# BenTheBacker/galvanise_zero

Hardware: AMD Instinct MI355X
Metric: self-play games/sec + NN leaf-evals/sec, breakthrough 8x8 @ 800 playouts/move (higher is better)
Workload: dtype bf16x3 split (hi+lo bf16 operands, ~16-bit significand, 3 MFMAs per product, fp32 accumulate)

## Files before the change

### galvanise_zero_amd/csrc/nn/forward_kernel.h

```cpp
#pragma once

#include <hip/hip_runtime.h>
#include <stdint.h>

#include <utility>

namespace gznn {

constexpr int kMaxRoles = 4;
constexpr int kMaxSegments = 32;
constexpr int kHeadBoards = 4;
constexpr int kMaxSE = 128;

struct Segment {
    int row0;
    const float* planes;
    float* pol[kMaxRoles];
    float* val;
};

typedef __attribute__((ext_vector_type(8))) __bf16 bf16x8;
typedef __attribute__((ext_vector_type(4))) float f32x4;

struct KParams {
    const __bf16* w0;
    const __bf16* w0lo;
    const float* b0;
    const __bf16* wres;
    const float* bres;
    const float* wh;
    const float* bh;
    const float* pd[kMaxRoles];
    const float* pb[kMaxRoles];
    const float* vhw;
    const float* vhb;
    const float* vdw;
    const float* vdb;
    const float* pre;
    const float* sew1;
    const float* sew2;
    float* feat;
    f32x4* resid;
    int n;
    int nseg;
    Segment seg[kMaxSegments];
    unsigned long long* stamps;
    int C, K0, B, R, VH, V, leaky, flatten_nchw, maxP, npos;
    int lgrow;
    int heads_seq;
    int H, W, wmagic;
    int value_sigmoid;
    int logits;
    int gemm_heads;
    const __bf16* pdp[kMaxRoles];
    int pkt;
    float* glog;
    int plog;
    int v2;
    int k0taps;
    int init_act;
    int S;
    int gapF;
    int FS;
    int btab_off;
    int se_off;
    int P[kMaxRoles];
    int VK;
    int cal;
    const float* wcl;
    const float* bcl;
    int cal_off;
    int nofuse;
};

__host__ __device__ constexpr int align16(int x) { return (x + 15) & ~15; }

template <int BPW, int NT = 256, bool BLOCKED = false>
__device__ __forceinline__ void dense_heads(const KParams& kp, const float* fk, float* lg, int board0, int nb);

constexpr int kMaxPTN = 23;
struct Board {
    int H, W, npos, wmagic;
    int tapmask[kMaxPTN];
    __device__ __forceinline__ int row(int p) const { return (p * wmagic) >> 16; }
};

constexpr bool kLoopSI = false;
constexpr bool kLoDirect = true;
constexpr bool kEpiInConv = false;

#ifndef GZ_STORE_SWAP
#define GZ_STORE_SWAP 0
#endif
constexpr bool kStoreSwap = GZ_STORE_SWAP != 0;

#ifndef GZ_H2_RING_VGPRS
#define GZ_H2_RING_VGPRS 128
#endif

__host__ __device__ constexpr int ring_depth(int nst, int ks, int ct, int cap) {
    const int cand[5] = {9, 6, 4, 3, 2};
    for (int i = 0; i < 5; ++i)
        if (nst % cand[i] == 0 && cand[i] * ks * ct * 4 <= cap && (cand[i] - 1) * ks * ct <= 60) return cand[i];
    return 1;
}

__host__ __device__ constexpr int gcd_c(int a, int b) { return b == 0 ? a : gcd_c(b, a % b); }
__host__ __device__ constexpr int lcm_c(int a, int b) { return a / gcd_c(a, b) * b; }

template <int F, int PTN, int NB = 1, int P = 1, int WG = 1>
struct Geo {
    static constexpr int P2 = P == 3 ? 2 : 1;
    static constexpr int WP = P == 1 ? 1 : 2;
    static constexpr int NPOS = 16 * PTN;
    static constexpr int PT = PTN;
    static constexpr int TT = NB * PT;
    static constexpr int NWV = WG == 3 ? 8 : (WG == 4 || WG == 5) ? 2 : 4;
    static constexpr int NGR = WG == 2 || WG == 4 || WG == 5 ? 2 : 1;
    static constexpr int CT = F / (16 * NWV);
    static constexpr int KC = F / 32;
    static constexpr int CPR = F / 8;
    static constexpr bool WRAP = CPR >= 16 && (P2 == 2 || PTN > 11);
    static constexpr int HALF = WRAP ? CPR * 16 : ((CPR + 14) * 16 + 255) & ~255;
    static constexpr int ROWS = WRAP ? P2 * HALF + 32 : P2 * HALF;
    static constexpr int ZROWS = WRAP ? 2 : 1;
    static constexpr int ACT_BYTES = (NPOS + ZROWS + 1) * ROWS;
    static constexpr int KS = (CT >= 4 || WP == 2) ? 1 : 2;
    static constexpr int NFR = CT * WP;
    static constexpr int ROWB = 64 * WP;
    static constexpr int NST = 9 * KC / KS;
    static constexpr int R0 = (P2 == 2 && (NB == 2 || WG == 2 || WG == 4 || WG == 5) && (KC / KS) >= 3 && NST % (KC / KS) == 0 &&
                               (KC / KS) * KS * NFR * 4 <= (WG == 4 ? GZ_H2_RING_VGPRS : WG == 5 ? 64 : 96))
                                  ? KC / KS
                                  : ring_depth(NST, KS, NFR, CT >= 4 ? 64 : 96);
    static constexpr int LIVE_VGPRS = R0 * KS * NFR * 4 + 2 * TT * P2 * 4 + 2 * CT * TT * 4;
    static constexpr bool SI = 2 * NB * ACT_BYTES + 16 * 1024 > 160 * 1024 || (NB == 1 && LIVE_VGPRS > 330) || P == 2;
    static constexpr int RS = ring_depth(NST, KS, NFR, 64);
    static constexpr int US = lcm_c(RS, KC / KS) * ((lcm_c(RS, KC / KS) * KS) % 2 ? 2 : 1);
    static constexpr bool LOOPSI = (kLoopSI || PTN > 11) && SI && NST % US == 0 && NST / US >= 2;
    static constexpr int R = LOOPSI ? RS : R0;
    static constexpr int LPS = KS * NFR;
    static constexpr bool INPL = WG == 5;
    static constexpr bool RG = CT * TT * 4 * 2 > 256;
    static constexpr bool TRACKED = SI || LIVE_VGPRS > 300 || (P2 == 2 && (NB == 2 || WG == 2 || WG == 4 || WG == 5));
    static_assert(F % 64 == 0, "filters must be a multiple of 64");
    static_assert(!SI || NB == 1, "single-image mode takes one board per workgroup");
    static_assert(WG == 1 || ((WG == 2 || WG == 4 || WG == 5) && NB == 1 && !SI) || (WG == 3 && !SI && CT >= 1),
                  "wave groups: two images, or one in place (INPL), never the single-image conv and heads");
    static_assert(!INPL || (P == 3 && WRAP), "in place: the split F = 128 kernels");
    static_assert(!RG || SI, "the global residual is implemented for single-image kernels");
    static constexpr int RESID_BYTES = RG ? 4 * CT * TT * 64 * 16 : 0;
    static constexpr int LO_BYTES = P == 2 ? ACT_BYTES : 0;
    static_assert(KC % KS == 0, "a stage must not straddle a tap");
    static_assert(R >= 2, "no ring depth fits");
    static constexpr int SPT = KC / KS;
    static constexpr int U0 = lcm_c(R, SPT);
    static constexpr int U = (U0 * KS) % 2 ? 2 * U0 : U0;
    static constexpr int NIT = NST / U;
    static constexpr int TPI = U * KS / KC;
    static constexpr bool LOOP = !SI && NST % U == 0 && NIT >= 2;
    static_assert(!LOOPSI || (NST % U == 0 && NIT >= 2), "single-image looped conv");
};

__device__ __forceinline__ int swz(int q) { return (2 * q) & 14; }

__host__ __device__ inline int trunk_scratch_bytes(int npos, int C, int K0, int R, int P2, int F) {
    const int in_stage = align16(C * npos * 4) + P2 * align16((npos + 1) * K0 * 2);
    const int hc = 2 * R + 1;
    const int heads = align16((F / 16) * hc * npos * 4);
    return in_stage > heads ? in_stage : heads;
}
__host__ __device__ inline int bias_table_bytes(int F, int B) { return align16((2 * B) * F * 4); }
__host__ __device__ inline int se_scratch_bytes(int F, int NB, int S) { return align16(NB * (F + S) * 4); }

__device__ __forceinline__ float act_fn(float v, int leaky) {
    return v > 0.f ? v : (leaky ? 0.03f * v : 0.f);
}
__device__ __forceinline__ float act_mx(float v, float alpha) { return fmaxf(v, alpha * v); }

__device__ __forceinline__ uint32_t pack2(float a, float b) {
    __bf16 x = (__bf16)a, y = (__bf16)b;
    return (uint32_t)__builtin_bit_cast(uint16_t, x) | ((uint32_t)__builtin_bit_cast(uint16_t, y) << 16);
}

__device__ __forceinline__ float bf16_lo(float x) { return x - (float)(__bf16)x; }

template <int F, int PTN, int P = 1, bool SEL = true>
__device__ __forceinline__ void store_act(char* X, int p, int co, f32x4 v, int npos) {
    using G = Geo<F, PTN, 1, P>;
    if constexpr (SEL && G::WRAP && kStoreSwap) {
        const int q = p >= npos ? npos + G::ZROWS : p;
        const uint32_t h0 = pack2(v[0], v[1]), h1 = pack2(v[2], v[3]);
        const uint32_t l0 = pack2(bf16_lo(v[0]), bf16_lo(v[1])), l1 = pack2(bf16_lo(v[2]), bf16_lo(v[3]));
        const auto s0 = __builtin_amdgcn_permlane16_swap(h0, l0, false, false);
        const auto s1 = __builtin_amdgcn_permlane16_swap(h1, l1, false, false);
        char* a = X + q * G::ROWS + ((co >> 3) << 4) + ((co & 4) ? G::HALF : 0);
        *(uint4*)a = uint4{s0[0], s1[0], s0[1], s1[1]};
        return;
    }
    if (SEL || p < npos) {
        const int q = SEL && p >= npos ? npos + G::ZROWS : p;
        const int chunk = G::WRAP ? (co >> 3) : ((co >> 3) + swz(q));
        char* a = X + q * G::ROWS + (chunk << 4) + (co & 7) * 2;
        uint2 u;
        if constexpr (P == 2) {
            u.x = pack2(bf16_lo(v[0]), bf16_lo(v[1]));
            u.y = pack2(bf16_lo(v[2]), bf16_lo(v[3]));
        } else {
            u.x = pack2(v[0], v[1]);
            u.y = pack2(v[2], v[3]);
        }
        *(uint2*)a = u;
        if constexpr (G::P2 == 2) {
            uint2 l;
            l.x = pack2(bf16_lo(v[0]), bf16_lo(v[1]));
            l.y = pack2(bf16_lo(v[2]), bf16_lo(v[3]));
            *(uint2*)(a + G::HALF) = l;
        }
    }
}

template <int F, int PTN>
__device__ __forceinline__ void store_lo_scratch(char* xlo, int p, int co, f32x4 v, int npos) {
    using G = Geo<F, PTN, 1, 2>;
    if (p < npos) {
        const int chunk = G::WRAP ? (co >> 3) : (co >> 3) + swz(p);
        uint2 l;
        l.x = pack2(bf16_lo(v[0]), bf16_lo(v[1]));
        l.y = pack2(bf16_lo(v[2]), bf16_lo(v[3]));
        *(uint2*)(xlo + p * G::ROWS + (chunk << 4) + (co & 7) * 2) = l;
    }
}

__device__ __forceinline__ float wave_sum(float v) {
#pragma unroll
    for (int o = 32; o > 0; o >>= 1) v += __shfl_xor(v, o, 64);
    return v;
}

__device__ __forceinline__ float wave_max(float v) {
#pragma unroll
    for (int o = 32; o > 0; o >>= 1) v = fmaxf(v, __shfl_xor(v, o, 64));
    return v;
}

__device__ __forceinline__ int find_segment(const KParams& kp, int board) {
    int s = 0;
    while (s + 1 < kp.nseg && board >= kp.seg[s + 1].row0) ++s;
    return s;
}

template <int IMM>
__device__ __forceinline__ bf16x8 gload_issue(uint32_t voff, const void* sbase) {
    bf16x8 v;
    asm volatile("global_load_dwordx4 %0, %1, %2 offset:%3" : "=v"(v) : "v"(voff), "s"(sbase), "n"(IMM) : "memory");
    return v;
}
template <int N>
__device__ __forceinline__ void ring_wait() { asm volatile("s_waitcnt vmcnt(%0)" ::"n"(N) : "memory"); }
__device__ __forceinline__ void ring_ready(bf16x8& v) { asm volatile("" : "+v"(v)); }


template <int F, int PTN, int NB, int P, int WG = 1>
struct Ring {
    using G = Geo<F, PTN, NB, P, WG>;
    bf16x8 r[G::R][G::KS][G::NFR];
};

template <int WP, int ROWB, int FR>
struct FragOff {
    static_assert(ROWB == 64 * WP, "16 rows x ROWB bytes = WP fragments of 1 KB");
    static constexpr int value = FR * 1024;
};
template <int F, int PTN, int NB, int P, int WG, int SLOT, int PARTS, int FR>
__device__ __forceinline__ void ring_issue_f(Ring<F, PTN, NB, P, WG>& ring, int k, uint32_t woff, const char* sb) {
    using G = Geo<F, PTN, NB, P, WG>;
    if constexpr ((PARTS >> (FR % G::WP)) & 1) {
        if constexpr (G::TRACKED)
            ring.r[SLOT][k][FR] = *(const bf16x8*)(sb + woff + FragOff<G::WP, G::ROWB, FR>::value);
        else
            ring.r[SLOT][k][FR] = gload_issue<FragOff<G::WP, G::ROWB, FR>::value>(woff, sb);
    }
}
template <int F, int PTN, int NB, int P, int WG, int SLOT, int PARTS, int... FRS>
__device__ __forceinline__ void ring_issue_k(Ring<F, PTN, NB, P, WG>& ring, int k, uint32_t woff, const char* sb,
                                             std::integer_sequence<int, FRS...>) {
    (ring_issue_f<F, PTN, NB, P, WG, SLOT, PARTS, FRS>(ring, k, woff, sb), ...);
}
template <int F, int PTN, int NB, int P, int WG, int SLOT, int PARTS = 3>
__device__ __forceinline__ void ring_issue(Ring<F, PTN, NB, P, WG>& ring, const __bf16* wres, uint32_t woff, int gs, int gmax) {
    using G = Geo<F, PTN, NB, P, WG>;
    int s = gs < gmax ? gs : gmax;
    if constexpr (P == 2) s = (s / (2 * G::NST)) * G::NST + s % G::NST;
#pragma unroll
    for (int k = 0; k < G::KS; ++k)
        ring_issue_k<F, PTN, NB, P, WG, SLOT, PARTS>(ring, k, woff, (const char*)wres + (size_t)(s * G::KS + k) * F * G::ROWB,
                                                    std::make_integer_sequence<int, G::NFR>{});
}

__device__ __forceinline__ void launder(int& v) { asm volatile("" : "+v"(v)); }
template <typename T>
__device__ __forceinline__ void launder_ptr(T*& p) { asm volatile("" : "+v"(p)); }
struct TapAddr {
    int row, rot;
};
template <int F, int PTN, int P = 1>
__device__ __forceinline__ TapAddr tap_base(int tap, int pt, int lane, const Board& bd) {
    using G = Geo<F, PTN, 1, P>;
    const int li = lane & 15, g = lane >> 4;
    const int dy = tap / 3 - 1, dx = tap % 3 - 1;
    const int p = 16 * pt + li;
    static_assert(PTN <= kMaxPTN, "board larger than the tap masks");
    const int qv = p + (dy * bd.W + dx);
    const bool ok = (bd.tapmask[pt] >> tap) & 1;
    if constexpr (G::WRAP) {
        const int a_in = qv * G::ROWS + (g << 4);
        const int a_zero = bd.npos * G::ROWS + (((g + swz(qv)) & 15) << 4);
        const int m = -(int)ok;
        return TapAddr{(a_in & m) | (a_zero & ~m), 0};
    }
    const int rot = (g + swz(qv)) << 4;
    return TapAddr{(ok ? qv : bd.npos) * G::ROWS, rot};
}
template <int F, int PTN, int P = 1>
__device__ __forceinline__ int tap_offset(const TapAddr& t, int kc) {
    return t.row + t.rot + 64 * kc;
}

template <int F, int PTN, int NB, int P, int WG, int PASS, int ST>
__device__ __forceinline__ void conv_stage(const char* __restrict__ X, Ring<F, PTN, NB, P, WG>& ring,
                                           f32x4 (&acc)[Geo<F, PTN, NB, P, WG>::CT][Geo<F, PTN, NB, P, WG>::TT],
                                           bf16x8 (&b)[2][Geo<F, PTN, NB, P, WG>::TT][Geo<F, PTN, NB, P, WG>::P2],
                                           const __bf16* wres, uint32_t woff, int gs0, int gmax, int& lane,
                                           const Board& bd) {
    using G = Geo<F, PTN, NB, P, WG>;
    constexpr int R = G::R, KS = G::KS, CT = G::CT, PT = G::PT, TT = G::TT, KC = G::KC, P2 = G::P2, WP = G::WP;
    constexpr bool next_in_pass = ST + R - 1 < G::NST;
    constexpr bool hi_only = P == 2 && G::TRACKED && (next_in_pass ? PASS == 1 : PASS == 0);
    ring_issue<F, PTN, NB, P, WG, (ST + R - 1) % R, hi_only ? 1 : 3>(ring, wres, woff, gs0 + ST + R - 1, gmax);
    if constexpr (!G::TRACKED) {
        ring_wait<(R - 1) * G::LPS>();
#pragma unroll
        for (int k = 0; k < KS; ++k)
#pragma unroll
            for (int f = 0; f < G::NFR; ++f) ring_ready(ring.r[ST % R][k][f]);
    }

#pragma unroll
    for (int k = 0; k < KS; ++k) {
        const int j = ST * KS + k;
        if (j + 1 < 9 * KC) {
            const int jn = j + 1;
            const int tap = jn / KC, kc = jn % KC;
            if (kc == 0) launder(lane);
#pragma unroll
            for (int pt = 0; pt < PT; ++pt) {
                const char* a = X + tap_offset<F, PTN, P>(tap_base<F, PTN, P>(tap, pt, lane, bd), kc);
#pragma unroll
                for (int bb = 0; bb < NB; ++bb)
#pragma unroll
                    for (int h = 0; h < P2; ++h)
                        b[jn & 1][bb * PT + pt][h] = *(const bf16x8*)(a + bb * G::ACT_BYTES + h * G::HALF);
            }
        }
#pragma unroll
        for (int ct = 0; ct < CT; ++ct)
#pragma unroll
            for (int t = 0; t < TT; ++t) {
                const bf16x8 w_hi = ring.r[ST % R][k][ct * WP];
                acc[ct][t] = __builtin_amdgcn_mfma_f32_16x16x32_bf16(w_hi, b[j & 1][t][0], acc[ct][t], 0, 0, 0);
                if constexpr (P == 3) {
                    const bf16x8 w_lo = ring.r[ST % R][k][ct * WP + 1];
                    acc[ct][t] = __builtin_amdgcn_mfma_f32_16x16x32_bf16(w_hi, b[j & 1][t][1], acc[ct][t], 0, 0, 0);
                    acc[ct][t] = __builtin_amdgcn_mfma_f32_16x16x32_bf16(w_lo, b[j & 1][t][0], acc[ct][t], 0, 0, 0);
                } else if constexpr (P == 2 && PASS == 0) {
                    const bf16x8 w_lo = ring.r[ST % R][k][ct * WP + 1];
                    acc[ct][t] = __builtin_amdgcn_mfma_f32_16x16x32_bf16(w_lo, b[j & 1][t][0], acc[ct][t], 0, 0, 0);
                }
            }
        if constexpr (!G::SI) {
#pragma unroll
            for (int t = 0; t < TT; ++t) {
                __builtin_amdgcn_sched_group_barrier(0x008, CT * (P2 == 2 ? 3 : 1), 0);
                __builtin_amdgcn_sched_group_barrier(0x100, P2, 0);
            }
        }
        __builtin_amdgcn_sched_barrier(0);
    }
}

template <int F, int PTN, int NB, int P, int WG, int... S>
__device__ __forceinline__ void ring_prime(Ring<F, PTN, NB, P, WG>& ring, const __bf16* wres, uint32_t woff, int gmax,
                                           std::integer_sequence<int, S...>) {
    (ring_issue<F, PTN, NB, P, WG, S>(ring, wres, woff, S, gmax), ...);
}

template <int F, int PTN, int NB, int P, int WG, int PASS, int... ST>
__device__ __forceinline__ void conv_stages(const char* __restrict__ X, Ring<F, PTN, NB, P, WG>& ring,
                                            f32x4 (&acc)[Geo<F, PTN, NB, P, WG>::CT][Geo<F, PTN, NB, P, WG>::TT],
                                            bf16x8 (&b)[2][Geo<F, PTN, NB, P, WG>::TT][Geo<F, PTN, NB, P, WG>::P2],
                                            const __bf16* wres, uint32_t woff, int gs0, int gmax, int& lane,
                                            const Board& bd, std::integer_sequence<int, ST...>) {
    (conv_stage<F, PTN, NB, P, WG, PASS, ST>(X, ring, acc, b, wres, woff, gs0, gmax, lane, bd), ...);
}

template <int F, int PTN, int NB, int P, int WG = 1, int PASS = 0>
__device__ __forceinline__ void conv3x3(const char* __restrict__ X, Ring<F, PTN, NB, P, WG>& ring,
                                        f32x4 (&acc)[Geo<F, PTN, NB, P, WG>::CT][Geo<F, PTN, NB, P, WG>::TT],
                                        const __bf16* wres, uint32_t woff, int gs0, int gmax, int lane,
                                        const Board& bd) {
    using G = Geo<F, PTN, NB, P, WG>;
    constexpr int PT = G::PT, TT = G::TT;
    if constexpr (PASS == 0) {
#pragma unroll
        for (int ct = 0; ct < G::CT; ++ct)
#pragma unroll
            for (int t = 0; t < TT; ++t) acc[ct][t] = f32x4{0.f, 0.f, 0.f, 0.f};
    }
    bf16x8 b[2][TT][G::P2];
    launder(lane);
#pragma unroll
    for (int pt = 0; pt < PT; ++pt) {
        const char* a = X + tap_offset<F, PTN, P>(tap_base<F, PTN, P>(0, pt, lane, bd), 0);
#pragma unroll
        for (int bb = 0; bb < NB; ++bb)
#pragma unroll
            for (int h = 0; h < G::P2; ++h) b[0][bb * PT + pt][h] = *(const bf16x8*)(a + bb * G::ACT_BYTES + h * G::HALF);
    }
    conv_stages<F, PTN, NB, P, WG, PASS>(X, ring, acc, b, wres, woff, gs0, gmax, lane, bd,
                                     std::make_integer_sequence<int, G::NST>{});
}

__device__ __forceinline__ void mfma_split3(f32x4& acc, const bf16x8& wh, const bf16x8& bh, const bf16x8& bl,
                                            const bf16x8& wl) {
    asm volatile(
        "v_mfma_f32_16x16x32_bf16 %0, %1, %2, %0\n\t"
        "v_mfma_f32_16x16x32_bf16 %0, %1, %3, %0\n\t"
        "v_mfma_f32_16x16x32_bf16 %0, %4, %2, %0"
        : "+a"(acc)
        : "v"(wh), "v"(bh), "v"(bl), "v"(wl));
}
template <int CT, int TT>
__device__ __forceinline__ void split_chain_enter(f32x4 (&acc)[CT][TT]) {
#pragma unroll
    for (int ct = 0; ct < CT; ++ct)
#pragma unroll
        for (int t = 0; t < TT; ++t) asm volatile("" : "+a"(acc[ct][t]));
    asm volatile("s_nop 1" ::: "memory");
}
template <int CT, int TT>
__device__ __forceinline__ void split_chain_leave(f32x4 (&acc)[CT][TT]) {
    asm volatile("s_nop 15\n\ts_nop 7" ::: "memory");
#pragma unroll
    for (int ct = 0; ct < CT; ++ct)
#pragma unroll
        for (int t = 0; t < TT; ++t) asm volatile("" : "+a"(acc[ct][t]));
}

struct NoEpi {
    __device__ __forceinline__ void operator()(int) const {}
};

template <int CT, int TT>
__device__ __forceinline__ void tile_leave(f32x4 (&acc)[CT][TT], int t) {
    asm volatile("s_nop 15\n\ts_nop 3" ::: "memory");
#pragma unroll
    for (int ct = 0; ct < CT; ++ct) asm volatile("" : "+a"(acc[ct][t]));
}

template <int F, int PTN, int NB, int P, int WG, int PASS, int ST, bool EPI = false, class Epi = NoEpi>
__device__ __forceinline__ void conv_stage_l(const char* __restrict__ X, Ring<F, PTN, NB, P, WG>& ring,
                                             f32x4 (&acc)[Geo<F, PTN, NB, P, WG>::CT][Geo<F, PTN, NB, P, WG>::TT],
                                             bf16x8 (&b)[Geo<F, PTN, NB, P, WG>::TT][Geo<F, PTN, NB, P, WG>::P2],
                                             const __bf16* wres, uint32_t woff, int gs_it, int gmax, int& lane,
                                             const Board& bd, int tap0, bool last_it, const Epi& epi = Epi{}) {
    using G = Geo<F, PTN, NB, P, WG>;
    constexpr int R = G::R, KS = G::KS, CT = G::CT, PT = G::PT, KC = G::KC, P2 = G::P2, WP = G::WP;
    static_assert(P != 2 || G::TRACKED, "two-pass split: compiler-tracked weight loads");
    static_assert(G::U % R == 0, "ring slots must be static within an iteration");
    if constexpr (P == 2) {
        constexpr int SLOT = (ST + R - 1) % R;
        const int gs = gs_it + ST + R - 1;
        ring_issue<F, PTN, NB, P, WG, SLOT, 1>(ring, wres, woff, gs, gmax);
        if constexpr (ST + R - 1 < G::U) {
            if constexpr (PASS == 0) ring_issue<F, PTN, NB, P, WG, SLOT, 2>(ring, wres, woff, gs, gmax);
        } else if ((PASS == 0) != last_it) {
            ring_issue<F, PTN, NB, P, WG, SLOT, 2>(ring, wres, woff, gs, gmax);
        }
    } else {
        ring_issue<F, PTN, NB, P, WG, (ST + R - 1) % R>(ring, wres, woff, gs_it + ST + R - 1, gmax);
    }
    if constexpr (!G::TRACKED) {
        ring_wait<(R - 1) * G::LPS>();
#pragma unroll
        for (int k = 0; k < KS; ++k)
#pragma unroll
            for (int f = 0; f < G::NFR; ++f) ring_ready(ring.r[ST % R][k][f]);
    }
#pragma unroll
    for (int k = 0; k < KS; ++k) {
        const int jn = ST * KS + k + 1;
        const int tap = tap0 + jn / KC, kc = jn % KC;
        if (kc == 0) launder(lane);
        int nb_off[PT];
#pragma unroll
        for (int pt = 0; pt < PT; ++pt) nb_off[pt] = tap_offset<F, PTN, P>(tap_base<F, PTN, P>(tap, pt, lane, bd), kc);
#pragma unroll
        for (int bb = 0; bb < NB; ++bb)
#pragma unroll
            for (int pt = 0; pt < PT; ++pt) {
                const int t = bb * PT + pt;
#pragma unroll
                for (int ct = 0; ct < CT; ++ct) {
                    const bf16x8 w_hi = ring.r[ST % R][k][ct * WP];
                    if constexpr (P2 == 2) {
                        mfma_split3(acc[ct][t], w_hi, b[t][0], b[t][1], ring.r[ST % R][k][ct * WP + 1]);
                    } else {
                        acc[ct][t] = __builtin_amdgcn_mfma_f32_16x16x32_bf16(w_hi, b[t][0], acc[ct][t], 0, 0, 0);
                        if constexpr (P == 2 && PASS == 0) {
                            const bf16x8 w_lo = ring.r[ST % R][k][ct * WP + 1];
                            acc[ct][t] = __builtin_amdgcn_mfma_f32_16x16x32_bf16(w_lo, b[t][0], acc[ct][t], 0, 0, 0);
                        }
                    }
                }
                {
                    const char* a = X + nb_off[pt] + bb * G::ACT_BYTES;
#pragma unroll
                    for (int h = 0; h < P2; ++h) b[t][h] = *(const bf16x8*)(a + h * G::HALF);
                }
                if constexpr (P2 == 1) {
                    __builtin_amdgcn_sched_group_barrier(0x008, CT * (P == 2 && PASS == 0 ? 2 : 1), 0);
                    __builtin_amdgcn_sched_group_barrier(0x100, P2, 0);
                }
                if constexpr (EPI && ST == G::U - 1) {
                    if (k == KS - 1 && t >= 1) {
                        if constexpr (P2 == 2) tile_leave(acc, t - 1);
                        epi(t - 1);
                    }
                }
            }
        if constexpr (EPI && ST == G::U - 1) {
            if (k == KS - 1) {
                if constexpr (P2 == 2) tile_leave(acc, G::TT - 1);
                epi(G::TT - 1);
            }
        }
        __builtin_amdgcn_sched_barrier(0);
    }
}

template <int F, int PTN, int NB, int P, int WG, int PASS, bool EPI, class Epi, int... ST>
__device__ __forceinline__ void conv_iter(const char* __restrict__ X, Ring<F, PTN, NB, P, WG>& ring,
                                          f32x4 (&acc)[Geo<F, PTN, NB, P, WG>::CT][Geo<F, PTN, NB, P, WG>::TT],
                                          bf16x8 (&b)[Geo<F, PTN, NB, P, WG>::TT][Geo<F, PTN, NB, P, WG>::P2],
                                          const __bf16* wres, uint32_t woff, int gs_it, int gmax, int& lane,
                                          const Board& bd, int tap0, bool last_it, const Epi& epi,
                                          std::integer_sequence<int, ST...>) {
    (conv_stage_l<F, PTN, NB, P, WG, PASS, ST, EPI, Epi>(X, ring, acc, b, wres, woff, gs_it, gmax, lane, bd, tap0, last_it,
                                                         epi), ...);
}

template <int F, int PTN, int NB, int P, int WG = 1, int PASS = 0, bool EPI = false, class Epi = NoEpi>
__device__ __forceinline__ void conv3x3_looped(const char* __restrict__ X, Ring<F, PTN, NB, P, WG>& ring,
                                               f32x4 (&acc)[Geo<F, PTN, NB, P, WG>::CT][Geo<F, PTN, NB, P, WG>::TT],
                                               const __bf16* wres, uint32_t woff, int gs0, int gmax, int lane,
                                               const Board& bd, const Epi& epi = Epi{}) {
    using G = Geo<F, PTN, NB, P, WG>;
    constexpr int PT = G::PT, TT = G::TT;
    if constexpr (PASS == 0) {
#pragma unroll
        for (int ct = 0; ct < G::CT; ++ct)
#pragma unroll
            for (int t = 0; t < TT; ++t) acc[ct][t] = f32x4{0.f, 0.f, 0.f, 0.f};
    }
    bf16x8 b[TT][G::P2];
    launder(lane);
#pragma unroll
    for (int pt = 0; pt < PT; ++pt) {
        const char* a = X + tap_offset<F, PTN, P>(tap_base<F, PTN, P>(0, pt, lane, bd), 0);
#pragma unroll
        for (int bb = 0; bb < NB; ++bb)
#pragma unroll
            for (int h = 0; h < G::P2; ++h) b[bb * PT + pt][h] = *(const bf16x8*)(a + bb * G::ACT_BYTES + h * G::HALF);
    }
    if constexpr (G::P2 == 2) split_chain_enter(acc);
    constexpr int NLOOP = EPI ? G::NIT - 1 : G::NIT;
#pragma clang loop unroll(disable)
    for (int it = 0; it < NLOOP; ++it)
        conv_iter<F, PTN, NB, P, WG, PASS, false, NoEpi>(X, ring, acc, b, wres, woff, gs0 + it * G::U, gmax, lane, bd,
                                                       it * G::TPI, it == G::NIT - 1, NoEpi{},
                                                       std::make_integer_sequence<int, G::U>{});
    if constexpr (EPI)
        conv_iter<F, PTN, NB, P, WG, PASS, true, Epi>(X, ring, acc, b, wres, woff, gs0 + NLOOP * G::U, gmax, lane, bd,
                                                   NLOOP * G::TPI, true, epi, std::make_integer_sequence<int, G::U>{});
    if constexpr (G::P2 == 2) split_chain_leave(acc);
}

template <int F, int PTN, int NB, int P, int WG = 1>
__device__ __forceinline__ f32x4 board_channel_sum(const f32x4 (&acc)[Geo<F, PTN, NB, P, WG>::CT][Geo<F, PTN, NB, P, WG>::TT],
                                                   int ct, int bb, int li, int npos) {
    using G = Geo<F, PTN, NB, P, WG>;
    f32x4 s = {0.f, 0.f, 0.f, 0.f};
#pragma unroll
    for (int pt = 0; pt < G::PT; ++pt)
        if (16 * pt + li < npos) {
            const f32x4 v = acc[ct][bb * G::PT + pt];
            s[0] += v[0]; s[1] += v[1]; s[2] += v[2]; s[3] += v[3];
        }
#pragma unroll
    for (int o = 1; o < 16; o <<= 1)
#pragma unroll
        for (int r = 0; r < 4; ++r) s[r] += __shfl_xor(s[r], o, 64);
    return s;
}

template <int F, int PTN, int NB, int P, bool ADDB>
__device__ __forceinline__ void se_gates(const KParams& kp,
                                         const f32x4 (&acc)[Geo<F, PTN, NB, P>::CT][Geo<F, PTN, NB, P>::TT],
                                         const float* bt, int blk, float* ses, int co_base, int lane,
                                         f32x4 (&gate)[Geo<F, PTN, NB, P>::CT][NB]) {
    using G = Geo<F, PTN, NB, P>;
    constexpr int CT = G::CT, PT = G::PT;
    const int g = lane >> 4, li = lane & 15, npos = kp.npos, S = kp.S;
    float* mean = ses;
    float* hid = ses + NB * F;
    const float inv = 1.f / (float)npos;
#pragma unroll
    for (int bb = 0; bb < NB; ++bb)
#pragma unroll
        for (int ct = 0; ct < CT; ++ct) {
            f32x4 s;
            if constexpr (ADDB) {
                const float4 bias = *(const float4*)(bt + co_base + 16 * ct + 4 * g);
                s = f32x4{0.f, 0.f, 0.f, 0.f};
#pragma unroll
                for (int pt = 0; pt < PT; ++pt)
                    if (16 * pt + li < npos) {
                        f32x4 v = acc[ct][bb * PT + pt];
                        v[0] += bias.x; v[1] += bias.y; v[2] += bias.z; v[3] += bias.w;
                        s[0] += v[0]; s[1] += v[1]; s[2] += v[2]; s[3] += v[3];
                    }
#pragma unroll
                for (int o = 1; o < 16; o <<= 1)
#pragma unroll
                    for (int r = 0; r < 4; ++r) s[r] += __shfl_xor(s[r], o, 64);
            } else {
                s = board_channel_sum<F, PTN, NB, P>(acc, ct, bb, li, npos);
            }
            if (li == 0)
                *(float4*)(mean + bb * F + co_base + 16 * ct + 4 * g) =
                    make_float4(s[0] * inv, s[1] * inv, s[2] * inv, s[3] * inv);
        }
    __syncthreads();
    const float* w1 = kp.sew1 + (size_t)blk * F * S;
    for (int i = threadIdx.x; i < NB * S; i += 256) {
        const int bb = i / S, j = i - bb * S;
        float h = 0.f;
#pragma unroll 16
        for (int c = 0; c < F; ++c) h += mean[bb * F + c] * w1[c * S + j];
        hid[bb * S + j] = fmaxf(h, 0.f);
    }
    __syncthreads();
    const float* w2 = kp.sew2 + (size_t)blk * S * F;
    f32x4 z[CT][NB];
#pragma unroll
    for (int ct = 0; ct < CT; ++ct)
#pragma unroll
        for (int bb = 0; bb < NB; ++bb) z[ct][bb] = f32x4{0.f, 0.f, 0.f, 0.f};
    const float* w2l = w2 + co_base + 4 * g;
#pragma unroll 4
    for (int j = 0; j < S; ++j) {
        float4 w[CT];
#pragma unroll
        for (int ct = 0; ct < CT; ++ct) w[ct] = *(const float4*)(w2l + (size_t)j * F + 16 * ct);
#pragma unroll
        for (int bb = 0; bb < NB; ++bb) {
            const float h = hid[bb * S + j];
#pragma unroll
            for (int ct = 0; ct < CT; ++ct) {
                z[ct][bb][0] += h * w[ct].x; z[ct][bb][1] += h * w[ct].y;
                z[ct][bb][2] += h * w[ct].z; z[ct][bb][3] += h * w[ct].w;
            }
        }
    }
#pragma unroll
    for (int ct = 0; ct < CT; ++ct)
#pragma unroll
        for (int bb = 0; bb < NB; ++bb)
            gate[ct][bb] = f32x4{1.f / (1.f + __expf(-z[ct][bb][0])), 1.f / (1.f + __expf(-z[ct][bb][1])),
                                 1.f / (1.f + __expf(-z[ct][bb][2])), 1.f / (1.f + __expf(-z[ct][bb][3]))};
}

template <int F, int PTN, int NB, int P>
__device__ __forceinline__ void squeeze_excite(const KParams& kp,
                                               f32x4 (&acc)[Geo<F, PTN, NB, P>::CT][Geo<F, PTN, NB, P>::TT], int blk,
                                               float* ses, int co_base, int lane) {
    using G = Geo<F, PTN, NB, P>;
    constexpr int CT = G::CT, PT = G::PT;
    f32x4 gate[CT][NB];
    se_gates<F, PTN, NB, P, false>(kp, acc, nullptr, blk, ses, co_base, lane, gate);
#pragma unroll
    for (int ct = 0; ct < CT; ++ct)
#pragma unroll
        for (int bb = 0; bb < NB; ++bb)
#pragma unroll
            for (int pt = 0; pt < PT; ++pt) {
                f32x4& v = acc[ct][bb * PT + pt];
                v[0] *= gate[ct][bb][0]; v[1] *= gate[ct][bb][1]; v[2] *= gate[ct][bb][2]; v[3] *= gate[ct][bb][3];
            }
}

__device__ __forceinline__ f32x4 pre_act(f32x4 v, const float4& sc, const float4& sh, int leaky) {
    v[0] = act_fn(v[0] * sc.x + sh.x, leaky);
    v[1] = act_fn(v[1] * sc.y + sh.y, leaky);
    v[2] = act_fn(v[2] * sc.z + sh.z, leaky);
    v[3] = act_fn(v[3] * sc.w + sh.w, leaky);
    return v;
}

template <int F, int PTN, bool LD>
__device__ __forceinline__ void lo_copy(char* X, char* xlo, int npos, int tid) {
    using G = Geo<F, PTN, 1, 2>;
    const int n16 = npos * G::ROWS / 16;
    uint4* img = (uint4*)X;
    uint4* glo = (uint4*)xlo;
    if constexpr (LD) {
        const int lane = tid & 63;
        for (int i0 = tid - lane; i0 < n16; i0 += 256) {
            if (i0 + lane < n16)
                __builtin_amdgcn_global_load_lds((const __attribute__((address_space(1))) void*)(glo + i0 + lane),
                                                 (__attribute__((address_space(3))) void*)(img + i0), 16, 0, 0);
        }
        asm volatile("s_waitcnt vmcnt(0)" ::: "memory");
    } else {
#pragma unroll 4
        for (int i = tid; i < n16; i += 256) glo[i] = img[i];
    }
}
template <int F, int PTN>
__device__ __forceinline__ void save_lo_write_hi(char* X, char* xlo, const f32x4 (&acc)[Geo<F, PTN, 1, 2>::CT][Geo<F, PTN, 1, 2>::TT],
                                                 int npos, int tid, int co_base, int li, int g) {
    using G = Geo<F, PTN, 1, 2>;
    lo_copy<F, PTN, false>(X, xlo, npos, tid);
    asm volatile("s_waitcnt lgkmcnt(0)\n\ts_barrier" ::: "memory");
#pragma unroll
    for (int ct = 0; ct < G::CT; ++ct)
#pragma unroll
        for (int t = 0; t < G::TT; ++t) store_act<F, PTN, 1, false>(X, 16 * t + li, co_base + 16 * ct + 4 * g, acc[ct][t], npos);
    __syncthreads();
}

template <int F, int PTN, int NB, int WPE, int P, bool V2, int WG = 1>
__device__ __forceinline__ void trunk_body(const KParams& kp) {
    using G = Geo<F, PTN, NB, P, WG>;
    static_assert(P == 1 || (P == 3 && (NB == 1 || G::WRAP) && (G::CT * G::TT <= 16 || G::SI)) || (P == 2 && G::SI && (!V2 || kLoDirect)),
                  "split precision: F <= 128 (F = 256: single image)");
    constexpr int P2 = G::P2;
    constexpr int IP2 = G::WP;
    constexpr int PT = G::PT, TT = G::TT, CT = G::CT, R = G::R, NWV = G::NWV, NGR = G::NGR, kThreads = 64 * NWV;
    const int NPOS = kp.npos, H = kp.H, W = kp.W;
    Board bd{H, W, NPOS, kp.wmagic, {}};
    {
        const int li = threadIdx.x & 15;
#pragma unroll
        for (int pt = 0; pt < PT; ++pt) {
            const int p = 16 * pt + li;
            const int r = bd.row(p), x = p - r * W;
            int m = 0;
#pragma unroll
            for (int tap = 0; tap < 9; ++tap) {
                const int y = r + tap / 3 - 1, xx = x + tap % 3 - 1;
                if (p < NPOS && (unsigned)y < (unsigned)H && (unsigned)xx < (unsigned)W) m |= 1 << tap;
            }
            bd.tapmask[pt] = m;
        }
    }
    constexpr int ACT = G::ACT_BYTES;

    constexpr bool SI = G::SI, RG = G::RG;
    extern __shared__ __attribute__((aligned(16))) char smem[];
    const int grp = NGR == 1 ? 0 : __builtin_amdgcn_readfirstlane((int)(threadIdx.x / kThreads));
    char* X0 = smem + grp * NB * ACT;
    constexpr bool INPL = G::INPL;
    char* X1 = SI ? smem : INPL ? X0 : smem + NGR * NB * ACT + grp * NB * ACT;
    char* SCR = X1;
    char* SCR0 = SI || INPL ? smem : smem + NGR * NB * ACT;
    float* btab = (float*)(smem + kp.btab_off);

    const int board0 = (blockIdx.x * NGR + grp) * NB;
    const int tid = threadIdx.x & (kThreads - 1);
#define GZ_STAMP(i) \
    if (kp.stamps && threadIdx.x == 0) kp.stamps[(size_t)blockIdx.x * 8 + (i)] = __builtin_amdgcn_s_memtime()
    GZ_STAMP(0);
    const int lane = tid & 63;
    const int wave = __builtin_amdgcn_readfirstlane(tid >> 6);
    const int g = lane >> 4, li = lane & 15;
    const int co_base = wave * (F / NWV);
    const int C = kp.C, K0 = kp.K0;

    constexpr int kPF = 4;
    const int nf4 = (C * NPOS) >> 2;
    const float* in_b[NB];
    bool vec_b[NB];
    float4 pf[NB][kPF];
#pragma unroll
    for (int bb = 0; bb < NB; ++bb) {
        const bool live = board0 + bb < kp.n;
        const int sg = find_segment(kp, board0 + bb);
        in_b[bb] = live ? kp.seg[sg].planes + (size_t)(board0 + bb - kp.seg[sg].row0) * C * NPOS : nullptr;
        vec_b[bb] = ((C * NPOS) & 3) == 0 && nf4 <= kPF * kThreads && ((uintptr_t)in_b[bb] & 15) == 0;
#pragma unroll
        for (int k = 0; k < kPF; ++k) {
            const int i4 = tid + k * kThreads;
            pf[bb][k] = (live && vec_b[bb] && i4 < nf4) ? ((const float4*)in_b[bb])[i4] : make_float4(0.f, 0.f, 0.f, 0.f);
        }
    }

    static_assert((F / NWV) % 16 == 0, "a wave's output channels are whole 16-channel weight blocks");
    const uint32_t woff = (uint32_t)((co_base >> 4) * G::WP * 1024 + 16 * lane);
    const int gmax = (P == 2 ? 4 : 2) * kp.B * G::NST - 1;
    Ring<F, PTN, NB, P, WG> ring;
    if (kp.B > 0) ring_prime<F, PTN, NB, P, WG>(ring, kp.wres, woff, gmax, std::make_integer_sequence<int, R - 1>{});

    f32x4 acc[CT][TT];
    f32x4 resid[RG ? 1 : CT][RG ? 1 : TT];
    f32x4* rg = RG ? kp.resid + ((size_t)(blockIdx.x * 4 + wave) * CT * TT) * 64 + lane : nullptr;
    char* xlo = P == 2 ? (char*)kp.resid + (size_t)gridDim.x * G::RESID_BYTES + (size_t)blockIdx.x * G::LO_BYTES : nullptr;

    float* calp = (float*)(smem + kp.cal_off);
    static_assert(!V2 || NWV == 4, "concat_all_layers partials: four waves per group");
    auto cal_partial = [&](int j, int bb, int li, int g) {
        float4 wv[CT];
#pragma unroll
        for (int ct = 0; ct < CT; ++ct) wv[ct] = *(const float4*)(kp.wcl + (size_t)j * F + co_base + 16 * ct + 4 * g);
#pragma unroll
        for (int pt = 0; pt < PT; ++pt) {
            float sum = 0.f;
#pragma unroll
            for (int ct = 0; ct < CT; ++ct) {
                const f32x4 a = acc[ct][bb * PT + pt];
                sum += a[0] * wv[ct].x;
                sum += a[1] * wv[ct].y;
                sum += a[2] * wv[ct].z;
                sum += a[3] * wv[ct].w;
            }
            sum += __shfl_xor(sum, 16, 64);
            sum += __shfl_xor(sum, 32, 64);
            const int p = 16 * pt + li;
            if (g == 0 && p < NPOS) calp[(wave * NB + bb) * NPOS + p] = sum;
        }
    };
    auto cal_reduce = [&](int j) {
        for (int i = tid; i < NB * NPOS; i += kThreads) {
            const int bb = i / NPOS, p = i - bb * NPOS;
            const int board = board0 + bb;
            if (board >= kp.n) continue;
            float sum = kp.bcl[j];
#pragma unroll
            for (int w = 0; w < 4; ++w) sum += calp[(w * NB + bb) * NPOS + p];
            kp.feat[(size_t)board * kp.FS + 2 * kp.R * NPOS + j * NPOS + p] = act_fn(sum, kp.leaky);
        }
    };

    for (int i = threadIdx.x; i < 2 * kp.B * F; i += kThreads * NGR) btab[i] = kp.bres[i];
    for (int i = tid; i < NB * G::ZROWS * G::ROWS / 4 && !INPL; i += kThreads) {
        const int bb = i / (G::ZROWS * G::ROWS / 4), j = i % (G::ZROWS * G::ROWS / 4);
        ((uint32_t*)(X0 + bb * ACT + NPOS * G::ROWS))[j] = 0u;
    }

    float* sin = (float*)SCR;
    char* IM = SCR + align16(C * NPOS * 4);
    const int imrow = K0 * 2;
    char* IMlo = IM + align16((NPOS + 1) * imrow);
    const int nch0 = K0 >> 3;
    const int imswz = ((nch0 & -nch0) < 16 ? (nch0 & -nch0) : 16) - 1;
    const int nk0 = K0 >> 5;
    auto load_w0 = [&](int s, bf16x8 (&x)[CT], bf16x8 (&xl)[CT]) {
#pragma unroll
        for (int ct = 0; ct < CT; ++ct) {
            const size_t o = ((size_t)(s * F + co_base + 16 * ct + li)) * 32 + 8 * g;
            x[ct] = *(const bf16x8*)(kp.w0 + o);
            if constexpr (IP2 == 2) xl[ct] = *(const bf16x8*)(kp.w0lo + o);
        }
    };
    bf16x8 a0[CT], alo0[CT];
    load_w0(0, a0, alo0);
#pragma unroll
    for (int bb = 0; bb < NB; ++bb) {
        const float* in = in_b[bb];
        if (vec_b[bb]) {
#pragma unroll
            for (int k = 0; k < kPF; ++k)
                if (tid + k * kThreads < nf4) ((float4*)sin)[tid + k * kThreads] = pf[bb][k];
        } else {
            for (int i = tid; i < C * NPOS; i += kThreads) sin[i] = in != nullptr ? in[i] : 0.f;
        }
        if (SI || bb == 0)
            for (int i = tid; i < IP2 * align16((NPOS + 1) * imrow) / 16; i += kThreads) ((uint4*)IM)[i] = uint4{0u, 0u, 0u, 0u};
        __syncthreads();
        const int T0 = kp.k0taps;
        for (int i = tid; i < NPOS * T0; i += kThreads) {
            int p = i, tap = 4;
            if (T0 == 9) { p = i / 9; tap = i - p * 9; }
            const int r = bd.row(p);
            const int y = r + tap / 3 - 1, x = p - r * W + tap % 3 - 1;
            if ((unsigned)y < (unsigned)H && (unsigned)x < (unsigned)W) {
                const float* src = sin + y * W + x;
                const int k0 = T0 == 9 ? tap * C : 0;
                for (int c = 0; c < C; ++c) {
                    const int k = k0 + c;
                    const int o = p * imrow + ((((k >> 3) ^ (p & imswz))) << 4) + (k & 7) * 2;
                    const float v = src[c * NPOS];
                    *(__bf16*)(IM + o) = (__bf16)v;
                    if constexpr (IP2 == 2) *(__bf16*)(IMlo + o) = (__bf16)bf16_lo(v);
                }
            }
        }
        __syncthreads();

#pragma unroll
        for (int ct = 0; ct < CT; ++ct)
#pragma unroll
            for (int pt = 0; pt < PT; ++pt) acc[ct][bb * PT + pt] = f32x4{0.f, 0.f, 0.f, 0.f};
        bf16x8 a[CT], alo[CT];
#pragma unroll
        for (int ct = 0; ct < CT; ++ct) {
            a[ct] = a0[ct];
            alo[ct] = alo0[ct];
        }
        for (int s = 0; s < nk0; ++s) {
            bf16x8 an[CT], alon[CT];
            if (s + 1 < nk0) load_w0(s + 1, an, alon);
#pragma unroll
            for (int pt = 0; pt < PT; ++pt) {
                const int p = 16 * pt + li;
                const int q = p < NPOS ? p : NPOS;
                const int o = q * imrow + ((((s * 4 + g)) ^ (q & imswz)) << 4);
                const bf16x8 bq = *(const bf16x8*)(IM + o);
#pragma unroll
                for (int ct = 0; ct < CT; ++ct) {
                    f32x4& c = acc[ct][bb * PT + pt];
                    c = __builtin_amdgcn_mfma_f32_16x16x32_bf16(a[ct], bq, c, 0, 0, 0);
                    if constexpr (IP2 == 2) {
                        const bf16x8 bql = *(const bf16x8*)(IMlo + o);
                        c = __builtin_amdgcn_mfma_f32_16x16x32_bf16(a[ct], bql, c, 0, 0, 0);
                        c = __builtin_amdgcn_mfma_f32_16x16x32_bf16(alo[ct], bq, c, 0, 0, 0);
                    }
                }
            }
            if (s + 1 < nk0) {
#pragma unroll
                for (int ct = 0; ct < CT; ++ct) {
                    a[ct] = an[ct];
                    if constexpr (IP2 == 2) alo[ct] = alon[ct];
                }
            }
        }
        if constexpr (SI || INPL) __syncthreads();
        const bool preact = V2 && kp.B > 0;
        f32x4* rg0 = rg;
        if constexpr (RG) launder_ptr(rg0);
        if constexpr (V2 && SI) {
            const bool bare = !kp.init_act;
#pragma unroll
            for (int ct = 0; ct < CT; ++ct) {
                const int co = co_base + 16 * ct + 4 * g;
                const float4 bias = *(const float4*)(kp.b0 + co);
                float4 psc = make_float4(1.f, 1.f, 1.f, 1.f), psh = make_float4(0.f, 0.f, 0.f, 0.f);
                if (preact) {
                    psc = *(const float4*)(kp.pre + co);
                    psh = *(const float4*)(kp.pre + F + co);
                }
#pragma unroll
                for (int pt = 0; pt < PT; ++pt) {
                    f32x4 v = acc[ct][bb * PT + pt];
                    v[0] += bias.x; v[1] += bias.y; v[2] += bias.z; v[3] += bias.w;
#pragma unroll
                    for (int r = 0; r < 4; ++r) {
                        const float a = act_fn(v[r], kp.leaky);
                        v[r] = ((int)bare | (int)(v[r] > 0.f)) ? v[r] : a;
                    }
                    if constexpr (RG) rg0[(ct * TT + bb * PT + pt) * 64] = v;
                    else resid[ct][bb * PT + pt] = v;
                    acc[ct][bb * PT + pt] = v;
                    const f32x4 sv = pre_act(v, psc, psh, kp.leaky);
                    if constexpr (P == 2) {
                        static_assert(P != 2 || kLoDirect, "two-pass v2: lo parts straight to the scratch");
                        store_act<F, PTN, 1, false>(X0 + bb * ACT, 16 * pt + li, co, sv, NPOS);
                        store_lo_scratch<F, PTN>(xlo, 16 * pt + li, co, sv, NPOS);
                    } else {
                        store_act<F, PTN, P, false>(X0 + bb * ACT, 16 * pt + li, co, sv, NPOS);
                    }
                }
            }
        } else
#pragma unroll
        for (int ct = 0; ct < CT; ++ct) {
            const int co = co_base + 16 * ct + 4 * g;
            const float4 bias = *(const float4*)(kp.b0 + co);
            float4 psc = make_float4(1.f, 1.f, 1.f, 1.f), psh = make_float4(0.f, 0.f, 0.f, 0.f);
            if (preact) {
                psc = *(const float4*)(kp.pre + co);
                psh = *(const float4*)(kp.pre + F + co);
            }
#pragma unroll
            for (int pt = 0; pt < PT; ++pt) {
                f32x4 v = acc[ct][bb * PT + pt];
                v[0] += bias.x; v[1] += bias.y; v[2] += bias.z; v[3] += bias.w;
                if (!V2 || kp.init_act) {
                    v[0] = act_fn(v[0], kp.leaky);
                    v[1] = act_fn(v[1], kp.leaky);
                    v[2] = act_fn(v[2], kp.leaky);
                    v[3] = act_fn(v[3], kp.leaky);
                }
                if constexpr (RG) rg0[(ct * TT + bb * PT + pt) * 64] = v;
                else resid[ct][bb * PT + pt] = v;
                acc[ct][bb * PT + pt] = v;
                if constexpr (P == 2 && kLoDirect) {
                    const f32x4 sv = preact ? pre_act(v, psc, psh, kp.leaky) : v;
                    store_act<F, PTN, 1, false>(X0 + bb * ACT, 16 * pt + li, co, sv, NPOS);
                    store_lo_scratch<F, PTN>(xlo, 16 * pt + li, co, sv, NPOS);
                } else {
                    store_act<F, PTN, P, !G::SI>(X0 + bb * ACT, 16 * pt + li, co, preact ? pre_act(v, psc, psh, kp.leaky) : v, NPOS);
                }
            }
        }
        if constexpr (V2)
            if (kp.cal) cal_partial(0, bb, li, g);
        __syncthreads();
        if constexpr (P == 2 && !kLoDirect) save_lo_write_hi<F, PTN>(X0, xlo, acc, NPOS, tid, co_base, li, g);
    }
    for (int i = tid; i < NB * G::ZROWS * G::ROWS / 4; i += kThreads) {
        const int bb = i / (G::ZROWS * G::ROWS / 4), j = i % (G::ZROWS * G::ROWS / 4);
        ((uint32_t*)(X1 + bb * ACT + NPOS * G::ROWS))[j] = 0u;
    }
    __syncthreads();
    if constexpr (V2)
        if (kp.cal) cal_reduce(0);

    GZ_STAMP(1);
    if constexpr (SI) {
        for (int cv = 0; cv < 2 * kp.B; ++cv) {
            const bool second = cv & 1;
            const float* bt = btab + cv * F;
            if constexpr (P == 2) {
                if constexpr (G::LOOPSI) conv3x3_looped<F, PTN, NB, P, WG, 0>(X0, ring, acc, kp.wres, woff, (2 * cv) * G::NST, gmax, lane, bd);
                else conv3x3<F, PTN, NB, P, WG, 0>(X0, ring, acc, kp.wres, woff, (2 * cv) * G::NST, gmax, lane, bd);
                __syncthreads();
                lo_copy<F, PTN, true>(X0, xlo, NPOS, tid);
                __syncthreads();
                if constexpr (G::LOOPSI) conv3x3_looped<F, PTN, NB, P, WG, 1>(X0, ring, acc, kp.wres, woff, (2 * cv + 1) * G::NST, gmax, lane, bd);
                else conv3x3<F, PTN, NB, P, WG, 1>(X0, ring, acc, kp.wres, woff, (2 * cv + 1) * G::NST, gmax, lane, bd);
            } else if constexpr (G::LOOPSI) {
                conv3x3_looped<F, PTN, NB, P, WG>(X0, ring, acc, kp.wres, woff, cv * G::NST, gmax, lane, bd);
            } else {
                conv3x3<F, PTN, NB, P, WG>(X0, ring, acc, kp.wres, woff, cv * G::NST, gmax, lane, bd);
            }
            __syncthreads();
            f32x4* rgc = rg;
            if constexpr (RG) launder_ptr(rgc);
            char* Xe = X0;
            launder_ptr(Xe);
            char* xloe = xlo;
            if constexpr (P == 2) launder_ptr(xloe);
            int lie = li, ge = g;
            launder(lie);
            launder(ge);
            if (V2 && second) {
                const int blk = cv >> 1;
                f32x4 gate[CT][NB];
#pragma unroll
                for (int ct = 0; ct < CT; ++ct)
#pragma unroll
                    for (int bb = 0; bb < NB; ++bb) gate[ct][bb] = f32x4{1.f, 1.f, 1.f, 1.f};
                if (kp.S)
                    se_gates<F, PTN, NB, P, true>(kp, acc, bt, blk, (float*)(smem + kp.se_off), co_base, 16 * ge + lie, gate);
                const bool more = blk + 1 < kp.B;
#pragma unroll
                for (int ct = 0; ct < CT; ++ct) {
                    const int co = co_base + 16 * ct + 4 * ge;
                    const float4 bias = *(const float4*)(bt + co);
                    float4 psc = make_float4(1.f, 1.f, 1.f, 1.f), psh = make_float4(0.f, 0.f, 0.f, 0.f);
                    if (more) {
                        psc = *(const float4*)(kp.pre + (size_t)(2 * blk + 2) * F + co);
                        psh = *(const float4*)(kp.pre + (size_t)(2 * blk + 3) * F + co);
                    }
#pragma unroll
                    for (int t = 0; t < TT; ++t) {
                        const f32x4 gt = gate[ct][t / PT];
                        f32x4 v = acc[ct][t], r;
                        v[0] += bias.x; v[1] += bias.y; v[2] += bias.z; v[3] += bias.w;
                        v[0] *= gt[0]; v[1] *= gt[1]; v[2] *= gt[2]; v[3] *= gt[3];
                        if constexpr (RG) r = rgc[(ct * TT + t) * 64];
                        else r = resid[ct][t];
                        v[0] += r[0]; v[1] += r[1]; v[2] += r[2]; v[3] += r[3];
                        if constexpr (RG) rgc[(ct * TT + t) * 64] = v;
                        else resid[ct][t] = v;
                        acc[ct][t] = v;
                        const f32x4 pv = pre_act(v, psc, psh, kp.leaky);
                        if constexpr (P == 2) {
                            store_act<F, PTN, 1, false>(Xe, 16 * t + lie, co, pv, NPOS);
                            store_lo_scratch<F, PTN>(xloe, 16 * t + lie, co, pv, NPOS);
                        } else {
                            store_act<F, PTN, P, !G::SI>(Xe, 16 * t + lie, co, pv, NPOS);
                        }
                    }
                }
                if (kp.cal)
#pragma unroll
                    for (int bb = 0; bb < NB; ++bb) cal_partial(blk + 1, bb, lie, ge);
                __syncthreads();
                if (kp.cal) cal_reduce(blk + 1);
                continue;
            }
#pragma unroll
            for (int ct = 0; ct < CT; ++ct) {
                const int co = co_base + 16 * ct + 4 * ge;
                const float4 bias = *(const float4*)(bt + co);
#pragma unroll
                for (int t = 0; t < TT; ++t) {
                    f32x4 v = acc[ct][t];
                    v[0] += bias.x; v[1] += bias.y; v[2] += bias.z; v[3] += bias.w;
                    if (second) {
                        f32x4 r;
                        if constexpr (RG) r = rgc[(ct * TT + t) * 64];
                        else r = resid[ct][t];
                        v[0] += r[0]; v[1] += r[1]; v[2] += r[2]; v[3] += r[3];
                    }
                    v[0] = act_fn(v[0], kp.leaky);
                    v[1] = act_fn(v[1], kp.leaky);
                    v[2] = act_fn(v[2], kp.leaky);
                    v[3] = act_fn(v[3], kp.leaky);
                    if (second) {
                        if constexpr (RG) rgc[(ct * TT + t) * 64] = v;
                        else resid[ct][t] = v;
                    }
                    if constexpr (P == 2 && kLoDirect) {
                        if (second) acc[ct][t] = v;
                        store_act<F, PTN, 1, false>(Xe, 16 * t + lie, co, v, NPOS);
                        store_lo_scratch<F, PTN>(xloe, 16 * t + lie, co, v, NPOS);
                    } else {
                        if (second || P == 2) acc[ct][t] = v;
                        store_act<F, PTN, P, !G::SI>(Xe, 16 * t + lie, co, v, NPOS);
                    }
                }
            }
            __syncthreads();
            if constexpr (P == 2 && !kLoDirect) save_lo_write_hi<F, PTN>(Xe, xlo, acc, NPOS, tid, co_base, lie, ge);
        }
    } else
    for (int blk = 0; blk < kp.B; ++blk) {
        const float alpha = kp.leaky ? 0.03f : 0.f;
        const float* b_a = btab + (2 * blk) * F;
        const float* b_b = b_a + F;

        static_assert(!(INPL && kEpiInConv), "an epilogue inside the conv writes the other image");
        if constexpr (!V2 && G::LOOP && kEpiInConv) {
            float4 bia[CT];
#pragma unroll
            for (int ct = 0; ct < CT; ++ct) bia[ct] = *(const float4*)(b_a + co_base + 16 * ct + 4 * g);
            auto epi1 = [&](int t) {
#pragma unroll
                for (int ct = 0; ct < CT; ++ct) {
                    f32x4 v = acc[ct][t];
                    v[0] = act_mx(v[0] + bia[ct].x, alpha);
                    v[1] = act_mx(v[1] + bia[ct].y, alpha);
                    v[2] = act_mx(v[2] + bia[ct].z, alpha);
                    v[3] = act_mx(v[3] + bia[ct].w, alpha);
                    store_act<F, PTN, P, !G::SI>(X1 + (t / PT) * ACT, 16 * (t % PT) + li, co_base + 16 * ct + 4 * g, v, NPOS);
                }
            };
            conv3x3_looped<F, PTN, NB, P, WG, 0, true>(X0, ring, acc, kp.wres, woff, (2 * blk) * G::NST, gmax, lane, bd, epi1);
            __syncthreads();
            float4 bib[CT];
#pragma unroll
            for (int ct = 0; ct < CT; ++ct) bib[ct] = *(const float4*)(b_b + co_base + 16 * ct + 4 * g);
            auto epi2 = [&](int t) {
#pragma unroll
                for (int ct = 0; ct < CT; ++ct) {
                    f32x4 v = acc[ct][t];
                    const f32x4 r = resid[ct][t];
                    v[0] = act_mx(v[0] + bib[ct].x + r[0], alpha);
                    v[1] = act_mx(v[1] + bib[ct].y + r[1], alpha);
                    v[2] = act_mx(v[2] + bib[ct].z + r[2], alpha);
                    v[3] = act_mx(v[3] + bib[ct].w + r[3], alpha);
                    resid[ct][t] = v;
                    acc[ct][t] = v;
                    store_act<F, PTN, P, !G::SI>(X0 + (t / PT) * ACT, 16 * (t % PT) + li, co_base + 16 * ct + 4 * g, v, NPOS);
                }
            };
            conv3x3_looped<F, PTN, NB, P, WG, 0, true>(X1, ring, acc, kp.wres, woff, (2 * blk + 1) * G::NST, gmax, lane, bd, epi2);
            __syncthreads();
            continue;
        }
        if constexpr (G::LOOP) conv3x3_looped<F, PTN, NB, P, WG>(X0, ring, acc, kp.wres, woff, (2 * blk) * G::NST, gmax, lane, bd);
        else conv3x3<F, PTN, NB, P, WG>(X0, ring, acc, kp.wres, woff, (2 * blk) * G::NST, gmax, lane, bd);
        if constexpr (INPL) __syncthreads();
#pragma unroll
        for (int ct = 0; ct < CT; ++ct) {
            const int co = co_base + 16 * ct + 4 * g;
            const float4 bias = *(const float4*)(b_a + co);
#pragma unroll
            for (int t = 0; t < TT; ++t) {
                f32x4 v = acc[ct][t];
                v[0] = act_mx(v[0] + bias.x, alpha);
                v[1] = act_mx(v[1] + bias.y, alpha);
                v[2] = act_mx(v[2] + bias.z, alpha);
                v[3] = act_mx(v[3] + bias.w, alpha);
                store_act<F, PTN, P, !G::SI>(X1 + (t / PT) * ACT, 16 * (t % PT) + li, co, v, NPOS);
            }
        }
        __syncthreads();

        if constexpr (G::LOOP) conv3x3_looped<F, PTN, NB, P, WG>(X1, ring, acc, kp.wres, woff, (2 * blk + 1) * G::NST, gmax, lane, bd);
        else conv3x3<F, PTN, NB, P, WG>(X1, ring, acc, kp.wres, woff, (2 * blk + 1) * G::NST, gmax, lane, bd);
        if constexpr (INPL) __syncthreads();
        if constexpr (V2) {
#pragma unroll
            for (int ct = 0; ct < CT; ++ct) {
                const float4 bias = *(const float4*)(b_b + co_base + 16 * ct + 4 * g);
#pragma unroll
                for (int t = 0; t < TT; ++t) {
                    acc[ct][t][0] += bias.x; acc[ct][t][1] += bias.y; acc[ct][t][2] += bias.z; acc[ct][t][3] += bias.w;
                }
            }
            if (kp.S) squeeze_excite<F, PTN, NB, P>(kp, acc, blk, (float*)(smem + kp.se_off), co_base, lane);
            const bool more = blk + 1 < kp.B;
#pragma unroll
            for (int ct = 0; ct < CT; ++ct) {
                const int co = co_base + 16 * ct + 4 * g;
                float4 psc = make_float4(1.f, 1.f, 1.f, 1.f), psh = make_float4(0.f, 0.f, 0.f, 0.f);
                if (more) {
                    psc = *(const float4*)(kp.pre + (size_t)(2 * blk + 2) * F + co);
                    psh = *(const float4*)(kp.pre + (size_t)(2 * blk + 3) * F + co);
                }
#pragma unroll
                for (int t = 0; t < TT; ++t) {
                    f32x4 v = acc[ct][t];
                    const f32x4 r = resid[ct][t];
                    v[0] += r[0]; v[1] += r[1]; v[2] += r[2]; v[3] += r[3];
                    resid[ct][t] = v;
                    acc[ct][t] = v;
                    if (more) store_act<F, PTN, P, !G::SI>(X0 + (t / PT) * ACT, 16 * (t % PT) + li, co, pre_act(v, psc, psh, kp.leaky), NPOS);
                }
            }
            if (kp.cal)
#pragma unroll
                for (int bb = 0; bb < NB; ++bb) cal_partial(blk + 1, bb, li, g);
            __syncthreads();
            if (kp.cal) cal_reduce(blk + 1);
            continue;
        }
#pragma unroll
        for (int ct = 0; ct < CT; ++ct) {
            const int co = co_base + 16 * ct + 4 * g;
            const float4 bias = *(const float4*)(b_b + co);
#pragma unroll
            for (int t = 0; t < TT; ++t) {
                f32x4 v = acc[ct][t];
                const f32x4 r = resid[ct][t];
                v[0] = act_mx(v[0] + bias.x + r[0], alpha);
                v[1] = act_mx(v[1] + bias.y + r[1], alpha);
                v[2] = act_mx(v[2] + bias.z + r[2], alpha);
                v[3] = act_mx(v[3] + bias.w + r[3], alpha);
                resid[ct][t] = v;
                acc[ct][t] = v;
                store_act<F, PTN, P, !G::SI>(X0 + (t / PT) * ACT, 16 * (t % PT) + li, co, v, NPOS);
            }
        }
        __syncthreads();
    }
    if constexpr (V2 && SI) {
#pragma unroll
        for (int ct = 0; ct < CT; ++ct)
#pragma unroll
            for (int t = 0; t < TT; ++t) {
                if constexpr (RG) acc[ct][t] = rg[(ct * TT + t) * 64];
                else acc[ct][t] = resid[ct][t];
            }
    }
    if (!G::TRACKED && kp.B > 0) {
        ring_wait<0>();
#pragma unroll
        for (int s = 0; s < R; ++s)
#pragma unroll
            for (int k = 0; k < G::KS; ++k)
#pragma unroll
                for (int f = 0; f < G::NFR; ++f) ring_ready(ring.r[s][k][f]);
    }

    GZ_STAMP(2);
    int lih = li, gh = g;
    if constexpr (V2 && SI) {
        launder(lih);
        launder(gh);
    }
    const int HC = 2 * kp.R + (kp.cal ? 0 : 1);
    constexpr int NT16 = F / 16;
    float* hpart = (float*)SCR;
    constexpr int kHoistHC = 5;
    constexpr bool HOIST_WH = !SI && CT <= 2;
    float4 whv[HOIST_WH ? kHoistHC : 1][CT];
    if constexpr (HOIST_WH) {
        if (HC <= kHoistHC) {
#pragma unroll
            for (int h = 0; h < kHoistHC; ++h)
#pragma unroll
                for (int ct = 0; ct < CT; ++ct)
                    if (h < HC) whv[h][ct] = *(const float4*)(kp.wh + (size_t)h * F + co_base + 16 * ct + 4 * gh);
        }
    }
    constexpr bool FUSE = !SI;
    const bool fuse = FUSE && !kp.nofuse;
    constexpr int NBW = NB * NGR;
    float* fk = (float*)(SCR0 + align16(NB * NT16 * HC * NPOS * 4));
    float* lg = fk + align16(kp.FS * NBW * 4) / 4;
    auto feat_at = [&](int bb, int k) -> float& {
        if (fuse) return fk[k * NBW + grp * NB + bb];
        return kp.feat[(size_t)(board0 + bb) * kp.FS + k];
    };
#pragma unroll
    for (int bb = 0; bb < NB; ++bb) {
        const int board = board0 + bb;
        if (kp.gapF && board < kp.n) {
            const float inv = 1.f / (float)NPOS;
#pragma unroll
            for (int ct = 0; ct < CT; ++ct) {
                const f32x4 sm = board_channel_sum<F, PTN, NB, P, WG>(acc, ct, bb, lih, NPOS);
                const int co = co_base + 16 * ct + 4 * gh;
                if (lih == 0)
#pragma unroll
                    for (int r = 0; r < 4; ++r)
                        if (co + r < kp.gapF) feat_at(bb, 2 * kp.R * NPOS + co + r) = sm[r] * inv;
            }
        }
        auto head_conv = [&](int h, const float4 (&wv)[CT]) {
#pragma unroll
            for (int pt = 0; pt < PT; ++pt) {
                const int p = 16 * pt + lih;
#pragma unroll
                for (int ct = 0; ct < CT; ++ct) {
                    const f32x4 a = acc[ct][bb * PT + pt];
                    float s = a[0] * wv[ct].x;
                    s += a[1] * wv[ct].y;
                    s += a[2] * wv[ct].z;
                    s += a[3] * wv[ct].w;
                    s += __shfl_xor(s, 16, 64);
                    s += __shfl_xor(s, 32, 64);
                    if (gh == 0 && p < NPOS) hpart[((bb * NT16 + co_base / 16 + ct) * HC + h) * NPOS + p] = s;
                }
            }
        };
        if constexpr (HOIST_WH) {
            if (HC <= kHoistHC) {
#pragma unroll
                for (int h = 0; h < kHoistHC; ++h)
                    if (h < HC) head_conv(h, whv[h]);
            }
        }
        if (!HOIST_WH || HC > kHoistHC) {
            for (int h = 0; h < HC; ++h) {
                float4 wv[CT];
#pragma unroll
                for (int ct = 0; ct < CT; ++ct) wv[ct] = *(const float4*)(kp.wh + (size_t)h * F + co_base + 16 * ct + 4 * gh);
                head_conv(h, wv);
            }
        }
    }
    __syncthreads();
    for (int i = tid; i < NB * HC * NPOS; i += kThreads) {
        const int bb = i / (HC * NPOS), hp = i - bb * (HC * NPOS);
        const int h = hp / NPOS, p = hp - h * NPOS;
        if (board0 + bb >= kp.n) continue;
        float s = kp.bh[h];
#pragma unroll
        for (int w = 0; w < NT16; ++w) s += hpart[((bb * NT16 + w) * HC + h) * NPOS + p];
        s = act_fn(s, kp.leaky);
        if (h < 2 * kp.R) {
            const int r = h >> 1, c = h & 1;
            const int idx = kp.flatten_nchw ? c * NPOS + p : p * 2 + c;
            feat_at(bb, r * 2 * NPOS + idx) = s;
        } else {
            feat_at(bb, 2 * kp.R * NPOS + kp.gapF + p) = s;
        }
    }
    __syncthreads();
    GZ_STAMP(3);
    if (fuse) {
        const int wb0 = blockIdx.x * NBW;
        const int nb = kp.n - wb0 < NBW ? kp.n - wb0 : NBW;
        dense_heads<NBW, kThreads * NGR>(kp, fk, lg, wb0, nb);
    }
    GZ_STAMP(4);
#undef GZ_STAMP
}

template <int F, int PTN, int NB, int WPE, int P>
__global__ void __launch_bounds__(256) __attribute__((amdgpu_waves_per_eu(WPE)))
trunk_kernel(const KParams kp) {
    trunk_body<F, PTN, NB, WPE, P, false>(kp);
}

template <int F, int PTN, int P>
__global__ void __launch_bounds__(512) __attribute__((amdgpu_waves_per_eu(2)))
trunk_kernel8(const KParams kp) {
    trunk_body<F, PTN, 1, 2, P, false, 2>(kp);
}

template <int F, int PTN, int P>
__global__ void __launch_bounds__(512) __attribute__((amdgpu_waves_per_eu(2)))
trunk_kernel_w8(const KParams kp) {
    trunk_body<F, PTN, 2, 2, P, false, 3>(kp);
}

template <int F, int PTN, int P>
__global__ void __launch_bounds__(256) __attribute__((amdgpu_waves_per_eu(1)))
trunk_kernel_h2(const KParams kp) {
    trunk_body<F, PTN, 1, 1, P, false, 4>(kp);
}

template <int F, int PTN, int P>
__global__ void __launch_bounds__(256) __attribute__((amdgpu_waves_per_eu(2)))
trunk_kernel_h2i(const KParams kp) {
    trunk_body<F, PTN, 1, 2, P, false, 5>(kp);
}

template <int F, int PTN, int NB, int WPE, int P>
__global__ void __launch_bounds__(256) __attribute__((amdgpu_waves_per_eu(WPE)))
trunk_kernel_v2(const KParams kp) {
    trunk_body<F, PTN, NB, WPE, P, true>(kp);
}

constexpr int kGemmSoftmaxMax = 3072;
constexpr int kDenseBlock = 64;

template <int BPW, int NT, bool BLOCKED = false>
__device__ __forceinline__ void dense_heads_seq(const KParams& kp, const float* fk, float* lg, int board0, int nb) {
    static_assert(BPW >= 1 && BPW <= 4, "one softmax wave per board");
    const int NPOS = kp.npos;
    const int LMAX = kp.lgrow;
    const int tid = threadIdx.x, lane = tid & 63, wave = tid >> 6;

    for (int r = 0; r < kp.R; ++r) {
        const int P = kp.P[r], K = 2 * NPOS;
        const float* Wd = kp.pd[r];
        const float* fr = fk + (size_t)r * 2 * NPOS * BPW;
        int lof = 0;
        for (int q = 0; q < r; ++q) lof += kp.P[q];
        if (kp.gemm_heads && P <= kGemmSoftmaxMax) {
            if (wave < nb) {
                constexpr int NV = kGemmSoftmaxMax / 64;
                const int b = wave, board = board0 + b;
                const float* l = kp.glog + (size_t)board * kp.plog + lof;
                float v[NV];
#pragma unroll
                for (int i = 0; i < NV; ++i) v[i] = lane + 64 * i < P ? l[lane + 64 * i] : -3.0e38f;
                float m = -3.0e38f;
#pragma unroll
                for (int i = 0; i < NV; ++i) m = fmaxf(m, v[i]);
                m = wave_max(m);
                float sum = 0.f;
#pragma unroll
                for (int i = 0; i < NV; ++i)
                    if (lane + 64 * i < P) sum += __expf(v[i] - m);
                sum = wave_sum(sum);
                const float inv = 1.f / sum;
                const int sg = find_segment(kp, board);
                float* out = kp.seg[sg].pol[r] + (size_t)(board - kp.seg[sg].row0) * P;
#pragma unroll
                for (int i = 0; i < NV; ++i)
                    if (lane + 64 * i < P) out[lane + 64 * i] = kp.logits ? v[i] : __expf(v[i] - m) * inv;
            }
            continue;
        }
        if (kp.gemm_heads) {
            for (int i = tid; i < nb * P; i += NT) {
                const int b = i / P, j = i - b * P;
                lg[b * LMAX + j] = kp.glog[(size_t)(board0 + b) * kp.plog + lof + j];
            }
        }
        for (int j = tid; j < P && !kp.gemm_heads; j += NT) {
            float a[BPW];
            float tot[BPW];
#pragma unroll
            for (int b = 0; b < BPW; ++b) a[b] = tot[b] = 0.f;
#pragma unroll 32
            for (int k = 0; k < K; ++k) {
                const float w = Wd[(size_t)k * ((P + 3) & ~3) + j];
#pragma unroll
                for (int b = 0; b < BPW; ++b) a[b] += fr[k * BPW + b] * w;
                if constexpr (BLOCKED)
                    if ((k & (kDenseBlock - 1)) == kDenseBlock - 1) {
#pragma unroll
                        for (int b = 0; b < BPW; ++b) { tot[b] += a[b]; a[b] = 0.f; }
                    }
            }
            if constexpr (BLOCKED) {
#pragma unroll
                for (int b = 0; b < BPW; ++b) a[b] = tot[b] + a[b];
            }
            const float bj = kp.pb[r][j];
#pragma unroll
            for (int b = 0; b < BPW; ++b) lg[b * LMAX + j] = a[b] + bj;
        }
        __syncthreads();
        if (wave < nb) {
            const int b = wave;
            const float* l = lg + b * LMAX;
            float m = -3.0e38f;
            for (int j = lane; j < P; j += 64) m = fmaxf(m, l[j]);
            m = wave_max(m);
            float sum = 0.f;
            for (int j = lane; j < P; j += 64) sum += __expf(l[j] - m);
            sum = wave_sum(sum);
            const float inv = 1.f / sum;
            const int board = board0 + b;
            const int sg = find_segment(kp, board);
            float* out = kp.seg[sg].pol[r] + (size_t)(board - kp.seg[sg].row0) * P;
            if (kp.logits) {
                for (int j = lane; j < P; j += 64) out[j] = l[j];
            } else {
                for (int j = lane; j < P; j += 64) out[j] = __expf(l[j] - m) * inv;
            }
        }
        __syncthreads();
    }

    {
        const int VH = kp.VH, VK = kp.VK;
        const float* fv = fk + (size_t)2 * kp.R * NPOS * BPW;
        for (int j = tid; j < VH; j += NT) {
            float a[BPW];
            float tot[BPW];
#pragma unroll
            for (int b = 0; b < BPW; ++b) a[b] = tot[b] = 0.f;
#pragma unroll 32
            for (int k = 0; k < VK; ++k) {
                const float w = kp.vhw[(size_t)k * ((VH + 3) & ~3) + j];
#pragma unroll
                for (int b = 0; b < BPW; ++b) a[b] += fv[k * BPW + b] * w;
                if constexpr (BLOCKED)
                    if ((k & (kDenseBlock - 1)) == kDenseBlock - 1) {
#pragma unroll
                        for (int b = 0; b < BPW; ++b) { tot[b] += a[b]; a[b] = 0.f; }
                    }
            }
            if constexpr (BLOCKED) {
#pragma unroll
                for (int b = 0; b < BPW; ++b) a[b] = tot[b] + a[b];
            }
            const float bj = kp.vhb[j];
#pragma unroll
            for (int b = 0; b < BPW; ++b) lg[b * LMAX + j] = act_fn(a[b] + bj, kp.leaky);
        }
        __syncthreads();
        if (wave < nb) {
            const int b = wave;
            const float* hv = lg + b * LMAX;
            float o[4] = {0.f, 0.f, 0.f, 0.f};
            for (int v = 0; v < kp.V; ++v) {
                float sum = 0.f;
                for (int k = lane; k < VH; k += 64) sum += hv[k] * kp.vdw[(size_t)k * kp.V + v];
                o[v] = wave_sum(sum) + kp.vdb[v];
            }
            if (lane == 0) {
                const int board = board0 + b;
                const int sg = find_segment(kp, board);
                float* out = kp.seg[sg].val + (size_t)(board - kp.seg[sg].row0) * kp.V;
                if (kp.logits) {
                    for (int v = 0; v < kp.V; ++v) out[v] = o[v];
                } else if (kp.value_sigmoid) {
                    for (int v = 0; v < kp.V; ++v) out[v] = 1.f / (1.f + __expf(-o[v]));
                } else {
                    float m = o[0];
                    for (int v = 1; v < kp.V; ++v) m = fmaxf(m, o[v]);
                    float e[4], esum = 0.f;
                    for (int v = 0; v < kp.V; ++v) { e[v] = __expf(o[v] - m); esum += e[v]; }
                    for (int v = 0; v < kp.V; ++v) out[v] = e[v] / esum;
                }
            }
        }
    }
}


template <int BPW, int NT, bool BLOCKED>
__device__ __forceinline__ void dense_heads(const KParams& kp, const float* fk, float* lg, int board0, int nb) {
    static_assert(BPW >= 1 && BPW <= 4, "one softmax wave per board");
    if (kp.heads_seq || (kp.gemm_heads && kp.maxP > kGemmSoftmaxMax)) {
        dense_heads_seq<BPW, NT, BLOCKED>(kp, fk, lg, board0, nb);
        return;
    }
    const int NPOS = kp.npos, R = kp.R, LG = kp.lgrow;
    const int tid = threadIdx.x, lane = tid & 63, wave = tid >> 6;
    const bool gem = kp.gemm_heads != 0;
    int pgroups = 0;
    if (!gem)
        for (int r = 0; r < R; ++r) pgroups += (kp.P[r] + 3) >> 2;
    const int VH4 = (kp.VH + 3) & ~3;
    const int voff = 4 * pgroups;
    const int units = pgroups + (VH4 >> 2);
    for (int u = tid; u < units; u += NT) {
        const float* W;
        const float* f;
        int K, N4, q, off, r = 0;
        if (u < pgroups) {
            int uu = u;
            off = 0;
            for (; r < R - 1; ++r) {
                const int g = (kp.P[r] + 3) >> 2;
                if (uu < g) break;
                uu -= g;
                off += 4 * g;
            }
            q = uu;
            W = kp.pd[r];
            N4 = (kp.P[r] + 3) & ~3;
            K = 2 * NPOS;
            f = fk + (size_t)r * 2 * NPOS * BPW;
        } else {
            q = u - pgroups;
            W = kp.vhw;
            N4 = VH4;
            K = kp.VK;
            f = fk + (size_t)2 * R * NPOS * BPW;
            off = voff;
        }
        float a[BPW][4];
        float tot[BPW][4];
#pragma unroll
        for (int b = 0; b < BPW; ++b) {
            a[b][0] = a[b][1] = a[b][2] = a[b][3] = 0.f;
            tot[b][0] = tot[b][1] = tot[b][2] = tot[b][3] = 0.f;
        }
        const float4* w4 = (const float4*)W + q;
        const int rs = N4 >> 2;
#pragma unroll 16
        for (int k = 0; k < K; ++k) {
            const float4 w = w4[(size_t)k * rs];
#pragma unroll
            for (int b = 0; b < BPW; ++b) {
                const float x = f[k * BPW + b];
                a[b][0] += x * w.x;
                a[b][1] += x * w.y;
                a[b][2] += x * w.z;
                a[b][3] += x * w.w;
            }
            if constexpr (BLOCKED)
                if ((k & (kDenseBlock - 1)) == kDenseBlock - 1) {
#pragma unroll
                    for (int b = 0; b < BPW; ++b)
#pragma unroll
                        for (int i = 0; i < 4; ++i) { tot[b][i] += a[b][i]; a[b][i] = 0.f; }
                }
        }
        if constexpr (BLOCKED) {
#pragma unroll
            for (int b = 0; b < BPW; ++b)
#pragma unroll
                for (int i = 0; i < 4; ++i) a[b][i] = tot[b][i] + a[b][i];
        }
        if (u < pgroups) {
#pragma unroll
            for (int i = 0; i < 4; ++i) {
                const int j = 4 * q + i;
                if (j < kp.P[r]) {
                    const float bj = kp.pb[r][j];
#pragma unroll
                    for (int b = 0; b < BPW; ++b) lg[b * LG + off + j] = a[b][i] + bj;
                }
            }
        } else {
#pragma unroll
            for (int i = 0; i < 4; ++i) {
                const int j = 4 * q + i;
                if (j < kp.VH) {
                    const float bj = kp.vhb[j];
#pragma unroll
                    for (int b = 0; b < BPW; ++b) lg[b * LG + off + j] = act_fn(a[b][i] + bj, kp.leaky);
                }
            }
        }
    }
    __syncthreads();
    const int ntask = R * nb + nb;
    for (int t = wave; t < ntask; t += NT / 64) {
        if (t < R * nb) {
            const int r = t / nb, b = t - r * nb, P = kp.P[r];
            int lof = 0;
            for (int q = 0; q < r; ++q) lof += gem ? kp.P[q] : ((kp.P[q] + 3) & ~3);
            const int board = board0 + b;
            const int sg = find_segment(kp, board);
            float* out = kp.seg[sg].pol[r] + (size_t)(board - kp.seg[sg].row0) * P;
            if (gem) {
                constexpr int NV = kGemmSoftmaxMax / 64;
                const float* l = kp.glog + (size_t)board * kp.plog + lof;
                float v[NV];
#pragma unroll
                for (int i = 0; i < NV; ++i) v[i] = lane + 64 * i < P ? l[lane + 64 * i] : -3.0e38f;
                float m = -3.0e38f;
#pragma unroll
                for (int i = 0; i < NV; ++i) m = fmaxf(m, v[i]);
                m = wave_max(m);
                float sum = 0.f;
#pragma unroll
                for (int i = 0; i < NV; ++i)
                    if (lane + 64 * i < P) sum += __expf(v[i] - m);
                sum = wave_sum(sum);
                const float inv = 1.f / sum;
#pragma unroll
                for (int i = 0; i < NV; ++i)
                    if (lane + 64 * i < P) out[lane + 64 * i] = kp.logits ? v[i] : __expf(v[i] - m) * inv;
            } else {
                const float* l = lg + b * LG + lof;
                float m = -3.0e38f;
                for (int j = lane; j < P; j += 64) m = fmaxf(m, l[j]);
                m = wave_max(m);
                float sum = 0.f;
                for (int j = lane; j < P; j += 64) sum += __expf(l[j] - m);
                sum = wave_sum(sum);
                const float inv = 1.f / sum;
                if (kp.logits) {
                    for (int j = lane; j < P; j += 64) out[j] = l[j];
                } else {
                    for (int j = lane; j < P; j += 64) out[j] = __expf(l[j] - m) * inv;
                }
            }
        } else {
            const int b = t - R * nb;
            const float* hv = lg + b * LG + voff;
            float o[4] = {0.f, 0.f, 0.f, 0.f};
            for (int v = 0; v < kp.V; ++v) {
                float sum = 0.f;
                for (int k = lane; k < kp.VH; k += 64) sum += hv[k] * kp.vdw[(size_t)k * kp.V + v];
                o[v] = wave_sum(sum) + kp.vdb[v];
            }
            if (lane == 0) {
                const int board = board0 + b;
                const int sg = find_segment(kp, board);
                float* out = kp.seg[sg].val + (size_t)(board - kp.seg[sg].row0) * kp.V;
                if (kp.logits) {
                    for (int v = 0; v < kp.V; ++v) out[v] = o[v];
                } else if (kp.value_sigmoid) {
                    for (int v = 0; v < kp.V; ++v) out[v] = 1.f / (1.f + __expf(-o[v]));
                } else {
                    float m = o[0];
                    for (int v = 1; v < kp.V; ++v) m = fmaxf(m, o[v]);
                    float e[4], esum = 0.f;
                    for (int v = 0; v < kp.V; ++v) { e[v] = __expf(o[v] - m); esum += e[v]; }
                    for (int v = 0; v < kp.V; ++v) out[v] = e[v] / esum;
                }
            }
        }
    }
}

__host__ __device__ inline int heads_row(int R, const int* P, int VH, bool two = true) {
    int maxP = 0, sum4 = 0;
    for (int r = 0; r < R; ++r) {
        maxP = P[r] > maxP ? P[r] : maxP;
        sum4 += (P[r] + 3) & ~3;
    }
    const int row = maxP > VH ? maxP : VH;
    const int tw = sum4 + ((VH + 3) & ~3);
    return two && tw > row ? tw : row;
}

__host__ __device__ inline int fused_heads_bytes(int npos, int R, int lgrow, int gapF, int nb, int nbg, int F) {
    const int FS = (2 * R + 1) * npos + gapF;
    return align16(nbg * (F / 16) * (2 * R + 1) * npos * 4) + align16(FS * nb * 4) + align16(nb * lgrow * 4);
}

#ifdef GZNN_DEFINE_HEADS_KERNEL
__global__ void __launch_bounds__(256) policy_gemm_kernel(const KParams kp) {
    const int r = blockIdx.z, P = kp.P[r], K = 2 * kp.npos;
    const int lane = threadIdx.x & 63, wave = threadIdx.x >> 6;
    const int jt0 = blockIdx.y * 8;
    const int njt = (P + 15) / 16;
    if (jt0 >= njt) return;
    const int board = blockIdx.x * 64 + wave * 16 + (lane & 15);
    const int kq = 8 * (lane >> 4);
    const float* f = kp.feat + (size_t)(board < kp.n ? board : 0) * kp.FS + (size_t)r * K;
    f32x4 acc[8];
#pragma unroll
    for (int t = 0; t < 8; ++t) acc[t] = f32x4{0.f, 0.f, 0.f, 0.f};
    const bf16x8* wp = (const bf16x8*)kp.pdp[r];
    for (int kt = 0; kt < kp.pkt; ++kt) {
        float x[8];
#pragma unroll
        for (int e = 0; e < 8; ++e) {
            const int k = 32 * kt + kq + e;
            x[e] = (board < kp.n && k < K) ? f[k] : 0.f;
        }
        bf16x8 bh, bl;
#pragma unroll
        for (int e = 0; e < 8; ++e) {
            bh[e] = (__bf16)x[e];
            bl[e] = (__bf16)(x[e] - (float)bh[e]);
        }
#pragma unroll
        for (int t = 0; t < 8; ++t) {
            const int jt = jt0 + t;
            if (jt < njt) {
                const size_t o = ((size_t)jt * kp.pkt + kt) * 128 + lane;
                const bf16x8 ah = wp[o], al = wp[o + 64];
                acc[t] = __builtin_amdgcn_mfma_f32_16x16x32_bf16(ah, bh, acc[t], 0, 0, 0);
                acc[t] = __builtin_amdgcn_mfma_f32_16x16x32_bf16(ah, bl, acc[t], 0, 0, 0);
                acc[t] = __builtin_amdgcn_mfma_f32_16x16x32_bf16(al, bh, acc[t], 0, 0, 0);
            }
        }
    }
    if (board >= kp.n) return;
    int lof = 0;
    for (int q = 0; q < r; ++q) lof += kp.P[q];
    float* out = kp.glog + (size_t)board * kp.plog + lof;
#pragma unroll
    for (int t = 0; t < 8; ++t) {
        const int j0 = (jt0 + t) * 16 + 4 * (lane >> 4);
#pragma unroll
        for (int i = 0; i < 4; ++i)
            if (j0 + i < P) out[j0 + i] = acc[t][i] + kp.pb[r][j0 + i];
    }
}

template <bool BLOCKED>
__device__ __forceinline__ void heads_body(const KParams& kp) {
    constexpr int BPW = kHeadBoards;
    extern __shared__ __attribute__((aligned(16))) float hs[];
    const int FS = kp.FS;
    float* fk = hs;
    float* lg = hs + FS * BPW;
    const int tid = threadIdx.x;
    const int board0 = blockIdx.x * BPW;
    const int nb = kp.n - board0 < BPW ? kp.n - board0 : BPW;
    for (int i0 = 0; i0 < BPW * FS; i0 += 8 * 256) {
        float r[8];
#pragma unroll
        for (int u = 0; u < 8; ++u) {
            const int i = i0 + u * 256 + tid;
            const int b = i / FS, k = i - b * FS;
            r[u] = (i < BPW * FS && b < nb) ? kp.feat[(size_t)(board0 + b) * FS + k] : 0.f;
        }
#pragma unroll
        for (int u = 0; u < 8; ++u) {
            const int i = i0 + u * 256 + tid;
            const int b = i / FS, k = i - b * FS;
            if (i < BPW * FS) fk[k * BPW + b] = r[u];
        }
    }
    __syncthreads();
    dense_heads<BPW, 256, BLOCKED>(kp, fk, lg, board0, nb);
}

__global__ void __launch_bounds__(256) heads_kernel(const KParams kp) { heads_body<false>(kp); }
__global__ void __launch_bounds__(256) heads_kernel_blocked(const KParams kp) { heads_body<true>(kp); }

#endif

__host__ inline int heads_lds_bytes(int FS, int lgrow) {
    return (FS * kHeadBoards + kHeadBoards * lgrow + kHeadBoards * 4) * 4;
}

}
```

### galvanise_zero_amd/csrc/nn/gz_nn.hip

```cpp
#define GZNN_DEFINE_HEADS_KERNEL
#include "forward_kernel.h"
#include "trunk_variants.h"
#include "fp32_forward.h"
#include "layered_forward.h"
#include "eval_cache.h"
#include "shadow_compare.h"
#include "symmetry.h"
#include "weight_image.h"
#include "../../../include/gzero_nn.h"

#include <hip/hip_runtime.h>

#include <algorithm>
#include <map>
#include <mutex>
#include <cmath>
#include <cstdio>
#include <cstdlib>
#include <cstring>
#include <string>
#include <vector>

using namespace gznn;
using namespace gzw;

static thread_local std::string g_err;

static int fail(const std::string& msg) {
    g_err = msg;
    return -1;
}

#define HIPCHK(x)                                                                        \
    do {                                                                                 \
        hipError_t e_ = (x);                                                             \
        if (e_ != hipSuccess) return fail(std::string(#x) + ": " + hipGetErrorString(e_)); \
    } while (0)


struct gz_net : PackSpec {
    int device = 0;
    size_t nweights = 0;
    struct Trunk {
        const void* fn = nullptr;
        int nb = 1;
        int smem = 0;
        int btab_off = 0;
        int se_off = 0;
        int cal_off = 0;
        bool fused_heads = false;
        int resid_bytes = 0;
        int threads = 256;
        int wgs_per_cu = 1;
        std::string name;
    } small, large;
    int large_min_rows = 1 << 30;
    bool has_weights = false;
    size_t image_bytes = 0;
    float last_roll_ms = 0.f;

    char* dmem = nullptr;
    KParams kp{};
    std::mutex wmu;
    unsigned long long wepoch = 1;

    hipStream_t stream = nullptr;
    hipEvent_t ev0 = nullptr, ev1 = nullptr;
    float* d_io = nullptr;
    int io_cap = 0;
    float last_ms = 0.f;
    int heads_smem = 0;
    std::map<hipStream_t, std::pair<float*, int>> glog;
    std::mutex feat_mu;
    std::map<hipStream_t, std::pair<float*, int>> feat;
    std::map<hipStream_t, std::pair<char*, size_t>> resid;
    unsigned long long* d_stamps = nullptr;
    int stamp_cap = 0;
    bool stamps_on = false;
    double stamp_avg[8] = {0};
    int chunk_rows = 1;
    const float* w0f = nullptr;
    const float* wresf = nullptr;
    std::map<hipStream_t, std::pair<char*, int>> fscr;
    int layered = 0;
    std::map<hipStream_t, int*> bexp;
    int in_width() const { return layered ? K0 : cp; }
    struct Shadow;
    Shadow* shadow = nullptr;
    std::mutex shadow_mu;
    bool is_shadow = false;
};

struct gz_net::Shadow {
    static constexpr int kSlots = 8;
    gz_net* net = nullptr;
    int every = 64, max_rows = 256;
    bool from_env = false;
    long forwards = 0;
    gz_shadow_stats* d_acc = nullptr;
    struct Out { float* out = nullptr; gzshadow::RowRecord* rec = nullptr; };
    std::map<hipStream_t, Out> out;
    struct Slot {
        gz_shadow_stats* host = nullptr;
        hipEvent_t e0 = nullptr, e1 = nullptr;
        bool pending = false;
        long epoch = 0;
    } slot[kSlots];
    int next = 0;
    hipStream_t last_stream = nullptr;
    int last_slot = -1;
    long epoch = 0;
    bool fresh = true;
    gz_shadow_stats done{};
};

extern "C" const char* gz_nn_last_error(void) { return g_err.c_str(); }


constexpr int kSmallVariant = 11, kLargeVariant = 23, kLargeFallback = 21, kLargeMinRows = 257;
constexpr int kLargeInPlace = 25;
constexpr int kCUs = 256;

static KernelChoice select_kernel(int fpad, int pt, int v, int precision, bool v2) {
    if (pt < 1 || pt > kMaxPT) return KernelChoice{};
    return trunk_variant(fpad, pt, v, precision, v2);
}

static gz_net* create_host(const gz_net_desc& d, int device, gz_net::Trunk* in_place) {
    if (d.cnn_kernel_size != 3) { fail("only cnn_kernel_size 3 is supported"); return nullptr; }
    if (d.role_count < 1 || d.role_count > GZ_MAX_ROLES) { fail("role_count out of range"); return nullptr; }
    if (d.num_values < 1 || d.num_values > 4) { fail("num_values out of range"); return nullptr; }
    if (initial_kernel(d) != 1 && initial_kernel(d) != 3) { fail("initial conv kernel must be 1 or 3"); return nullptr; }
    if (d.se_units < 0 || d.se_units > kMaxSE || (d.se_units && !d.resnet_v2)) {
        fail("squeeze-excite units must be 0.." + std::to_string(kMaxSE) + " on a v2 net");
        return nullptr;
    }
    if (d.concat_all_layers && (!d.resnet_v2 || d.global_pooling_value || d.value_bn)) {
        fail("concat_all_layers needs a v2 net without the pooling value head (model.py:251-252)");
        return nullptr;
    }
    const int precision = d.precision == 0 ? GZ_PRECISION_BF16 : d.precision;
    const bool fp32 = precision == GZ_PRECISION_FP32;
    const int layered = precision == GZ_PRECISION_BF16_LAYERED ? 1 : precision == GZ_PRECISION_SPLIT_LAYERED ? 3 :
                        precision == GZ_PRECISION_F16X3_LAYERED ? gzlayered::kF16Parts : 0;
    const bool layerwise = fp32 || layered;
    if (precision != GZ_PRECISION_BF16 && precision != GZ_PRECISION_SPLIT && !layerwise) { fail("unknown precision"); return nullptr; }
    int vs = kSmallVariant, vl = kLargeVariant, min_large = kLargeMinRows;
    if (const char* e = getenv("GZ_KERNEL_VARIANT")) {
        vs = vl = atoi(e);
        min_large = 1 << 30;
    }
    const int npos_ = d.input_columns * d.input_rows;
    const int pt = kernel_tiles((npos_ + 15) / 16);
    const int fpad = fp32 ? gzfp32::padded_filters(d.cnn_filter_size) : kernel_filters(d.cnn_filter_size, (npos_ + 15) / 16);
    if (d.input_rows > 32 || npos_ >= 1024) { fail("board too large"); return nullptr; }
    const bool v2 = d.resnet_v2 != 0;
    if (layerwise) {
        if (d.input_columns < 1 || d.input_rows < 1 || d.input_columns > gzfp32::kMaxBoardSide ||
            d.input_rows > gzfp32::kMaxBoardSide || fpad == 0 || d.input_channels < 1) {
            fail("unsupported network geometry F=" + std::to_string(d.cnn_filter_size) + " H=" +
                 std::to_string(d.input_columns) + " W=" + std::to_string(d.input_rows) +
                 (fp32 ? " (fp32-ieee: boards up to 19 x 19, F <= 256)" : " (layered modes: boards up to 19 x 19, F <= 256)"));
            return nullptr;
        }
        min_large = 1 << 30;
    }
    KernelChoice kc = layerwise ? KernelChoice{} : select_kernel(fpad, pt, vs, precision, v2);
    KernelChoice kl = layerwise ? KernelChoice{} : select_kernel(fpad, pt, vl, precision, v2);
    if (!kl.fn && vl == kLargeVariant) kl = select_kernel(fpad, pt, kLargeFallback, precision, v2);
    auto wg_fits = [&](const KernelChoice& c) {
        if (c.groups == 1) return true;
        const int np = d.input_columns * d.input_rows;
        const int kk0 = initial_kernel(d);
        const int k0p = ((kk0 * kk0 * d.input_channels + 31) / 32) * 32;
        const int p2 = precision == GZ_PRECISION_SPLIT ? 2 : 1;
        return trunk_scratch_bytes(np, d.input_channels, k0p, d.role_count, p2, fpad) <= c.act_bytes &&
               fused_heads_bytes(np, d.role_count, heads_row(d.role_count, d.policy_dist_count, d.value_hidden_size),
                                 gap_features(d), c.nb, 1, fpad) <= c.act_bytes;
    };
    if (kl.fn && !wg_fits(kl)) {
        kl = vl == kLargeVariant ? select_kernel(fpad, pt, kLargeFallback, precision, v2) : KernelChoice{};
        if (kl.fn && !wg_fits(kl)) kl = KernelChoice{};
    }
    if (kc.fn && !wg_fits(kc)) kc = KernelChoice{};
    KernelChoice ki = !layerwise && getenv("GZ_KERNEL_VARIANT") == nullptr && kl.fn
                          ? select_kernel(fpad, pt, kLargeInPlace, precision, v2) : KernelChoice{};
    if (ki.fn && !wg_fits(ki)) ki = KernelChoice{};
    if (kc.fn && !kl.fn && vl != vs) {
        kl = kc;
        min_large = 1 << 30;
    }
    if (!layerwise && (!kc.fn || !kl.fn)) {
        fail("unsupported network geometry F=" + std::to_string(d.cnn_filter_size) + " H=" +
             std::to_string(d.input_columns) + " W=" + std::to_string(d.input_rows) +
             (precision == GZ_PRECISION_SPLIT ? " (split precision)" : "") + (v2 ? " (v2)" : "") +
             (fpad == 256 ? " (F > 128: boards of up to 176 positions; larger boards run in fp32-ieee)" : ""));
        return nullptr;
    }
    gz_net* net = new gz_net;
    net->d = d;
    net->device = device;
    net->large_min_rows = min_large;
    static_cast<PackSpec&>(*net) = pack_spec(d, precision, fpad, false);
    net->layered = layered;
    const int k0 = initial_kernel(d);
    if (layerwise) {
        net->chunk_rows = gzfp32::chunk_rows_for(npos_, net->in_width(), fpad);
        if (const char* e = getenv("GZ_FP32_CHUNK_ROWS"))
            net->chunk_rows = std::max(1, std::min(atoi(e), net->chunk_rows));
    }
    net->nweights = blob_plan(d).consumed;
    int maxP = 0;
    for (int r = 0; r < d.role_count; ++r) maxP = std::max(maxP, d.policy_dist_count[r]);
    const int npos = d.input_columns * d.input_rows;
    int lgrow = heads_row(d.role_count, d.policy_dist_count, d.value_hidden_size, true);
    bool heads_seq = false;
    const int scr_in = trunk_scratch_bytes(npos, d.input_channels, net->K0, d.role_count, net->p2, fpad);
    auto trunk = [&](const KernelChoice& c) {
        gz_net::Trunk t;
        t.fn = c.fn;
        t.nb = c.nb;
        t.threads = c.threads;
        t.wgs_per_cu = c.wgs_per_cu;
        t.name = c.name;
        t.fused_heads = !c.single_image && !d.concat_all_layers;
        const int scr = t.fused_heads ? std::max(scr_in, fused_heads_bytes(npos, d.role_count, lgrow, gap_features(d), c.nb,
                                                                           c.groups == 2 ? 1 : c.nb, fpad))
                                      : scr_in;
        t.btab_off = c.single_image ? align16(std::max(c.act_bytes, scr))
                     : c.in_place   ? c.nb * c.act_bytes
                                    : c.nb * c.act_bytes + std::max(c.nb * c.act_bytes, scr);
        t.resid_bytes = c.resid_bytes;
        t.smem = t.btab_off + bias_table_bytes(fpad, d.residual_layers);
        t.se_off = t.smem;
        if (d.se_units) t.smem += se_scratch_bytes(fpad, c.nb, d.se_units);
        t.cal_off = t.smem;
        if (d.concat_all_layers) t.smem += align16(4 * c.nb * npos * 4);
        return t;
    };
    const int FS = 2 * d.role_count * npos + value_features(d);
    for (int pass = 0; pass < 2; ++pass) {
        net->small = trunk(kc);
        net->large = trunk(kl);
        if (layerwise) {
            gz_net::Trunk t;
            t.name = layered ? gzlayered::conv_kernel_name(fpad, layered) : gzfp32::conv_kernel_name(fpad);
            net->small = net->large = t;
        }
        net->heads_smem = heads_lds_bytes(FS, lgrow);
        if (pass == 1 || (net->small.smem <= 160 * 1024 && net->large.smem <= 160 * 1024 && net->heads_smem <= 160 * 1024))
            break;
        heads_seq = true;
        lgrow = heads_row(d.role_count, d.policy_dist_count, d.value_hidden_size, false);
    }
    net->gemm_heads = !fp32 && !net->f16 && !net->small.fused_heads && !net->large.fused_heads && maxP >= 512 &&
                      getenv("GZ_NO_GEMM_HEADS") == nullptr;
    KParams& kp = net->kp;
    kp.C = d.input_channels;
    kp.K0 = net->K0;
    kp.B = d.residual_layers;
    kp.R = d.role_count;
    kp.VH = d.value_hidden_size;
    kp.V = d.num_values;
    kp.leaky = d.leaky_relu;
    kp.flatten_nchw = d.flatten_nchw;
    kp.value_sigmoid = d.value_sigmoid;
    kp.v2 = d.resnet_v2 ? 1 : 0;
    kp.k0taps = k0 * k0;
    kp.init_act = has_initial_bn(d) ? 1 : 0;
    kp.S = d.se_units;
    kp.gapF = gap_features(d);
    kp.FS = FS;
    kp.VK = value_features(d);
    kp.cal = cal_layers(d);
    kp.nofuse = d.concat_all_layers ? 1 : 0;
    kp.maxP = maxP;
    kp.lgrow = lgrow;
    kp.heads_seq = heads_seq ? 1 : 0;
    kp.npos = npos;
    kp.gemm_heads = net->gemm_heads ? 1 : 0;
    kp.pkt = (2 * npos + 31) / 32;
    kp.plog = 0;
    for (int r = 0; r < d.role_count; ++r) kp.plog += d.policy_dist_count[r];
    kp.H = d.input_columns;
    kp.W = d.input_rows;
    kp.wmagic = (65536 + kp.W - 1) / kp.W;
    for (int r = 0; r < d.role_count; ++r) kp.P[r] = d.policy_dist_count[r];

    for (const gz_net::Trunk* t : {&net->small, &net->large}) {
        if (t->smem > 160 * 1024) {
            fail("network needs " + std::to_string(t->smem) + " B of LDS per workgroup (160 KB max): too many residual blocks "
                 "for this board in this mode");
            delete net;
            return nullptr;
        }
    }
    *in_place = ki.fn && net->large_min_rows < (1 << 30) ? trunk(ki) : gz_net::Trunk{};
    return net;
}

static gz_net* create_device(gz_net* net, const gz_net::Trunk& in_place) {
    const int device = net->device;
    if (hipSetDevice(device) != hipSuccess || hipStreamCreateWithFlags(&net->stream, hipStreamNonBlocking) != hipSuccess ||
        hipEventCreate(&net->ev0) != hipSuccess || hipEventCreate(&net->ev1) != hipSuccess) {
        fail(std::string("HIP init failed: ") + hipGetErrorString(hipGetLastError()));
        delete net;
        return nullptr;
    }
    auto resident = [&](const gz_net::Trunk& t) {
        int nblk = 0;
        if (t.smem > 64 * 1024 && hipFuncSetAttribute(t.fn, hipFuncAttributeMaxDynamicSharedMemorySize, t.smem) != hipSuccess)
            return 0;
        if (hipOccupancyMaxActiveBlocksPerMultiprocessor(&nblk, t.fn, t.threads, t.smem) != hipSuccess) return 0;
        return nblk;
    };
    if (in_place.fn) {
        const gz_net::Trunk& t = in_place;
        if (2 * t.smem <= 160 * 1024 && resident(t) >= t.wgs_per_cu) net->large = t;
    }
    for (gz_net::Trunk* t : {&net->small, &net->large}) {
        if (t->smem > 64 * 1024 &&
            hipFuncSetAttribute(t->fn, hipFuncAttributeMaxDynamicSharedMemorySize, t->smem) != hipSuccess) {
            fail("cannot raise dynamic LDS limit");
            delete net;
            return nullptr;
        }
        if (t->wgs_per_cu > 1) t->wgs_per_cu = std::max(1, std::min(t->wgs_per_cu, resident(*t)));
    }
    if (net->heads_smem > 64 * 1024 &&
        hipFuncSetAttribute(net->fp32 || net->f16 ? (const void*)&heads_kernel_blocked : (const void*)&heads_kernel,
                            hipFuncAttributeMaxDynamicSharedMemorySize, net->heads_smem) != hipSuccess) {
        fail("cannot raise dynamic LDS limit (heads)");
        delete net;
        return nullptr;
    }
    return net;
}

namespace {
int net_precision(const gz_net_desc& d) { return d.precision == 0 ? GZ_PRECISION_BF16 : d.precision; }

gz_net* shadow_host(const gz_net_desc& d, int device, int precision, int every, int max_rows, gz_net::Trunk* in_place) {
    if (precision == 0) precision = GZ_PRECISION_BF16;
    if (precision == net_precision(d)) {
        fail("shadow: precision " + std::to_string(precision) + " is the net's own mode");
        return nullptr;
    }
    if (every < 1 || max_rows < 1) {
        fail("shadow: every and max_rows must be at least 1");
        return nullptr;
    }
    gz_net_desc sd = d;
    sd.precision = precision;
    gz_net* s = create_host(sd, device, in_place);
    if (!s) {
        fail("shadow: " + g_err);
        return nullptr;
    }
    s->is_shadow = true;
    return s;
}

int shadow_env(int* precision, int* every, int* max_rows) {
    const char* e = getenv("GZ_NN_SHADOW");
    if (!e || !*e) return 0;
    long v[3] = {0, 64, 256};
    int got = 0;
    const char* p = e;
    bool ok = true;
    while (ok && got < 3) {
        char* end = nullptr;
        const long x = strtol(p, &end, 10);
        ok = end != p && x >= 0 && x <= (1 << 20);
        v[got++] = x;
        p = end;
        if (!ok || *p == 0) break;
        ok = *p == ':' && got < 3;
        ++p;
    }
    if (!ok || *p != 0 || v[1] < 1 || v[2] < 1) {
        fail(std::string("GZ_NN_SHADOW: expected <precision>[:<every>[:<max_rows>]] with every and max_rows >= 1, got \"") + e + "\"");
        return -1;
    }
    *precision = (int)v[0];
    *every = (int)v[1];
    *max_rows = (int)v[2];
    return 1;
}

void shadow_free(gz_net::Shadow* sh) {
    if (!sh) return;
    if (sh->net) gz_net_destroy(sh->net);
    if (sh->d_acc) (void)hipFree(sh->d_acc);
    for (auto& o : sh->out) (void)hipFree(o.second.out);
    for (auto& s : sh->slot) {
        if (s.host) (void)hipHostFree(s.host);
        if (s.e0) (void)hipEventDestroy(s.e0);
        if (s.e1) (void)hipEventDestroy(s.e1);
    }
    delete sh;
}

int shadow_attach(gz_net* net, gz_net* s, const gz_net::Trunk& in_place, int every, int max_rows, bool from_env) {
    if (!create_device(s, in_place)) return fail("shadow: " + g_err);
    gz_net::Shadow* sh = new gz_net::Shadow;
    sh->net = s;
    sh->every = every;
    sh->max_rows = max_rows;
    sh->from_env = from_env;
    s->kp.logits = net->kp.logits;
    hipError_t e = hipMalloc((void**)&sh->d_acc, sizeof(gz_shadow_stats));
    for (auto& sl : sh->slot) {
        if (e == hipSuccess) e = hipHostMalloc((void**)&sl.host, sizeof(gz_shadow_stats), hipHostMallocDefault);
        if (e == hipSuccess) e = hipEventCreate(&sl.e0);
        if (e == hipSuccess) e = hipEventCreate(&sl.e1);
    }
    if (e != hipSuccess) {
        shadow_free(sh);
        return fail(std::string("shadow: ") + hipGetErrorString(e));
    }
    std::lock_guard<std::mutex> wl(net->wmu);
    std::lock_guard<std::mutex> sl(net->shadow_mu);
    net->shadow = sh;
    return 0;
}

void shadow_harvest(gz_net::Shadow* sh, int wait_slot = -1) {
    if (wait_slot >= 0 && sh->slot[wait_slot].pending) (void)hipEventSynchronize(sh->slot[wait_slot].e1);
    for (int k = 0; k < gz_net::Shadow::kSlots; ++k) {
        gz_net::Shadow::Slot& s = sh->slot[(sh->next + k) % gz_net::Shadow::kSlots];
        if (!s.pending) continue;
        if (hipEventQuery(s.e1) != hipSuccess) break;
        s.pending = false;
        if (s.epoch != sh->epoch) continue;
        float ms = 0.f;
        (void)hipEventElapsedTime(&ms, s.e0, s.e1);
        const double total = sh->done.device_ms + (double)ms;
        sh->done = *s.host;
        sh->done.device_ms = total;
    }
}
}

extern "C" gz_net* gz_net_create(const gz_net_desc* desc, int device) {
    if (!desc) { fail("null desc"); return nullptr; }
    gz_net::Trunk in_place, s_in_place;
    gz_net* net = create_host(*desc, device, &in_place);
    if (!net) return nullptr;
    gz_net* s = nullptr;
    int sp = 0, every = 0, max_rows = 0;
    const int env = shadow_env(&sp, &every, &max_rows);
    if (env > 0) s = shadow_host(*desc, device, sp, every, max_rows, &s_in_place);
    if (env < 0 || (env > 0 && !s)) {
        delete net;
        return nullptr;
    }
    net = create_device(net, in_place);
    if (!net) {
        delete s;
        return nullptr;
    }
    if (s && shadow_attach(net, s, s_in_place, every, max_rows, true)) {
        const std::string msg = g_err;
        gz_net_destroy(net);
        g_err = msg;
        return nullptr;
    }
    return net;
}

extern "C" size_t gz_shadow_stats_sizeof(void) { return sizeof(gz_shadow_stats); }

extern "C" int gz_net_shadow_enable(gz_net* net, int precision, int every, int max_rows) {
    if (!net) return fail("null net");
    if (net->is_shadow) return fail("shadow: a shadow cannot have a shadow of its own");
    {
        std::lock_guard<std::mutex> sl(net->shadow_mu);
        if (net->shadow) return fail("shadow: the net already has a shadow");
    }
    gz_net::Trunk in_place;
    gz_net* s = shadow_host(net->d, net->device, precision, every, max_rows, &in_place);
    if (!s) return -1;
    return shadow_attach(net, s, in_place, every, max_rows, false);
}

extern "C" int gz_net_shadow_disable(gz_net* net) {
    if (!net) return fail("null net");
    gz_net::Shadow* sh = nullptr;
    {
        std::lock_guard<std::mutex> wl(net->wmu);
        std::lock_guard<std::mutex> sl(net->shadow_mu);
        sh = net->shadow;
        net->shadow = nullptr;
    }
    if (!sh) return fail("shadow: the net has no shadow");
    HIPCHK(hipSetDevice(net->device));
    HIPCHK(hipDeviceSynchronize());
    shadow_free(sh);
    return 0;
}

extern "C" int gz_net_shadow_stats(gz_net* net, gz_shadow_stats* out, int reset) {
    if (!net || !out) return fail("null argument");
    std::lock_guard<std::mutex> sl(net->shadow_mu);
    gz_net::Shadow* sh = net->shadow;
    if (!sh) return fail("shadow: the net has no shadow");
    shadow_harvest(sh);
    *out = sh->done;
    if (reset) {
        ++sh->epoch;
        sh->fresh = true;
        sh->done = gz_shadow_stats{};
    }
    return 0;
}

extern "C" void gz_net_destroy(gz_net* net) {
    if (!net) return;
    (void)hipSetDevice(net->device);
    if (gz_net::Shadow* sh = net->shadow) {
        (void)hipDeviceSynchronize();
        if (sh->from_env) {
            shadow_harvest(sh);
            const gz_shadow_stats& t = sh->done;
            const long ok = t.rows - t.nonfinite_rows;
            fprintf(stderr,
                    "gz_nn shadow (precision %d vs %d, every %d, max_rows %d): checks %ld rows %ld nonfinite_rows %ld "
                    "max_abs_dp %.6g mean_abs_dp %.6g max_row_kl %.6g mean_row_kl %.6g argmax_mismatch %ld of %ld "
                    "max_abs_dv %.6g mean_abs_dv %.6g worst check %ld row %ld device_ms %.3f\n",
                    net_precision(net->d), net_precision(sh->net->d), sh->every, sh->max_rows, t.checks, t.rows, t.nonfinite_rows,
                    t.max_abs_dp, t.policy_elems ? t.sum_abs_dp / t.policy_elems : 0.0, t.max_row_kl,
                    t.policy_rows ? t.sum_row_kl / t.policy_rows : 0.0, t.argmax_mismatch, ok * net->d.role_count, t.max_abs_dv,
                    t.value_elems ? t.sum_abs_dv / t.value_elems : 0.0, t.worst_check, t.worst_row, t.device_ms);
        }
        net->shadow = nullptr;
        shadow_free(sh);
    }
    if (net->dmem) (void)hipFree(net->dmem);
    if (net->d_io) (void)hipFree(net->d_io);
    if (net->d_stamps) (void)hipFree(net->d_stamps);
    for (auto& f : net->feat) (void)hipFree(f.second.first);
    for (auto& f : net->resid) (void)hipFree(f.second.first);
    for (auto& f : net->glog) (void)hipFree(f.second.first);
    for (auto& f : net->fscr) (void)hipFree(f.second.first);
    for (auto& f : net->bexp) (void)hipFree(f.second);
    if (net->ev0) (void)hipEventDestroy(net->ev0);
    if (net->ev1) (void)hipEventDestroy(net->ev1);
    if (net->stream) (void)hipStreamDestroy(net->stream);
    delete net;
}

extern "C" size_t gz_net_weight_count(const gz_net* net) { return net ? net->nweights : 0; }

extern "C" int gz_net_heads_fused(const gz_net* net) { return net->large.fused_heads ? 1 : 0; }
extern "C" int gz_net_heads_path(const gz_net* net) {
    return (net->small.fused_heads ? GZ_HEADS_FUSED_SMALL : 0) | (net->large.fused_heads ? GZ_HEADS_FUSED_LARGE : 0) |
           (net->kp.heads_seq ? GZ_HEADS_SEQ : 0) | (net->gemm_heads ? GZ_HEADS_GEMM : 0) |
           (net->kp.maxP > kGemmSoftmaxMax ? GZ_HEADS_LONG_ROW : 0);
}

extern "C" double gz_net_flops_per_eval(const gz_net* net) {
    const gz_net_desc& d = net->d;
    const double F = d.cnn_filter_size, C = d.input_channels, HW = (double)d.input_columns * d.input_rows;
    const double k0 = initial_kernel(d);
    double f = 2 * HW * C * F * k0 * k0 + d.residual_layers * 2 * (2 * HW * F * F * 9);
    f += d.residual_layers * 2.0 * (2 * F * d.se_units);
    for (int r = 0; r < d.role_count; ++r) f += 2 * HW * F * 2 + 2 * (2 * HW) * d.policy_dist_count[r];
    f += 2 * HW * F * std::max(1, cal_layers(d)) + 2.0 * value_features(d) * d.value_hidden_size +
         2.0 * d.value_hidden_size * d.num_values;
    return f;
}

namespace {
char* swap_image(gz_net* net, char* m, const ImageLayout& I) {
    const int R = net->d.role_count;
    char* old = net->dmem;
    net->dmem = m;
    KParams& kp = net->kp;
    kp.w0 = (const __bf16*)(m + I.w0);
    kp.w0lo = (const __bf16*)(m + I.w0lo);
    kp.b0 = (const float*)(m + I.b0);
    kp.wres = (const __bf16*)(m + I.wres);
    net->w0f = (const float*)(m + I.w0);
    net->wresf = (const float*)(m + I.wres);
    kp.bres = (const float*)(m + I.bres);
    kp.wh = (const float*)(m + I.wh);
    kp.bh = (const float*)(m + I.bh);
    kp.wcl = (const float*)(m + I.wcl);
    kp.bcl = (const float*)(m + I.bcl);
    for (int r = 0; r < R; ++r) {
        kp.pd[r] = (const float*)(m + I.pd[r]);
        kp.pb[r] = (const float*)(m + I.pb[r]);
    }
    kp.vhw = (const float*)(m + I.vhw);
    kp.vhb = (const float*)(m + I.vhb);
    kp.vdw = (const float*)(m + I.vdw);
    kp.vdb = (const float*)(m + I.vdb);
    kp.pre = (const float*)(m + I.pre);
    kp.sew1 = (const float*)(m + I.sew1);
    kp.sew2 = (const float*)(m + I.sew2);
    for (int r = 0; r < R; ++r) kp.pdp[r] = net->gemm_heads ? (const __bf16*)(m + I.pdp[r]) : nullptr;
    net->has_weights = true;
    net->image_bytes = I.total;
    return old;
}

int install_image(gz_net* net, char* m, const ImageLayout& I, char* sm = nullptr, const ImageLayout* sI = nullptr) {
    std::unique_lock<std::mutex> wl(net->wmu);
    char* old = swap_image(net, m, I);
    ++net->wepoch;
    char* sold = nullptr;
    if (sm && net->shadow) {
        sold = swap_image(net->shadow->net, sm, *sI);
    } else if (sm) {
        sold = sm;
    }
    wl.unlock();
    if (old || sold) {
        HIPCHK(hipDeviceSynchronize());
        if (old) HIPCHK(hipFree(old));
        if (sold) HIPCHK(hipFree(sold));
    }
    return 0;
}

gz_net* shadow_of(gz_net* net) {
    if (!net || net->is_shadow) return nullptr;
    std::lock_guard<std::mutex> sl(net->shadow_mu);
    return net->shadow ? net->shadow->net : nullptr;
}

int check_count(const gz_net* net, const float* blob, size_t count) {
    if (!net || !blob) return fail("null argument");
    if (count != net->nweights)
        return fail("weight count mismatch: got " + std::to_string(count) + " expected " + std::to_string(net->nweights));
    return 0;
}

__global__ void fold_kernel(const BNRef* folds, const float* blob, float* fold) {
    const BNRef b = folds[blockIdx.x];
    for (int i = threadIdx.x; i < b.n; i += blockDim.x) fold_element(b, i, blob, fold);
}
__global__ void pack_kernel(const Job* jobs, const float* blob, const float* fold, char* image) {
    const Job j = jobs[blockIdx.y];
    const size_t n = j.count();
    for (size_t i = (size_t)blockIdx.x * blockDim.x + threadIdx.x; i < n; i += (size_t)gridDim.x * blockDim.x)
        pack_element(j.kind, j, (int)(i / j.cols), (int)(i % j.cols), blob, fold, RawImage{image});
}
}

static int build_image_host(gz_net* net, const float* blob, size_t count, char** mp, ImageLayout* Ip) {
    if (check_count(net, blob, count)) return -1;
    const ImageLayout I = image_layout(*net);
    std::vector<char> img(I.total, 0);
    const JobList J = job_list(*net, blob_plan(net->d), I);
    if (net->f16) {
        const int conv = f16_range_check(J, blob);
        if (conv >= 0)
            return fail((conv == 0 ? std::string("initial conv") : "trunk conv " + std::to_string(conv - 1) + " (residual block " +
                                                                     std::to_string((conv - 1) / 2) + ")") +
                        ": a BN-folded weight is outside fp16's finite range (|w| >= 65,520): fp16x3-layered cannot hold it");
    }
    pack_image_host(J, blob, RawImage{img.data()});
    HIPCHK(hipSetDevice(net->device));
    char* m = nullptr;
    HIPCHK(hipMalloc((void**)&m, I.total));
    if (hipMemcpy(m, img.data(), I.total, hipMemcpyHostToDevice) != hipSuccess) {
        (void)hipFree(m);
        return fail("weight upload failed");
    }
    *mp = m;
    *Ip = I;
    return 0;
}

extern "C" int gz_net_set_weights(gz_net* net, const float* blob, size_t count) {
    char *m = nullptr, *sm = nullptr;
    ImageLayout I, sI;
    if (build_image_host(net, blob, count, &m, &I)) return -1;
    if (gz_net* s = shadow_of(net)) {
        if (build_image_host(s, blob, count, &sm, &sI)) {
            (void)hipFree(m);
            return fail("shadow: " + g_err);
        }
    }
    return install_image(net, m, I, sm, &sI);
}

static int build_image_device(gz_net* net, const float* d_blob, size_t count, char** mp, ImageLayout* Ip) {
    const ImageLayout I = image_layout(*net);
    const JobList J = job_list(*net, blob_plan(net->d), I);
    HIPCHK(hipSetDevice(net->device));
    HIPCHK(hipDeviceSynchronize());
    hipStream_t st = net->stream;
    hipEvent_t e0, e1;
    HIPCHK(hipEventCreate(&e0));
    HIPCHK(hipEventCreate(&e1));
    HIPCHK(hipEventRecord(e0, st));
    char* m = nullptr;
    char* scratch = nullptr;
    auto cleanup = [&]() {
        if (scratch) (void)hipFree(scratch);
        (void)hipEventDestroy(e0);
        (void)hipEventDestroy(e1);
    };
    auto bail = [&](const std::string& what, hipError_t e) {
        cleanup();
        if (m) (void)hipFree(m);
        return fail(what + ": " + hipGetErrorString(e));
    };
    const size_t fold_bytes = ((size_t)J.fold_floats * 4 + 15) & ~(size_t)15;
    const size_t folds_bytes = (J.folds.size() * sizeof(BNRef) + 15) & ~(size_t)15, packs_bytes = J.packs.size() * sizeof(Job);
    hipError_t e;
    if ((e = hipMalloc((void**)&m, I.total)) != hipSuccess) return bail("hipMalloc image", e);
    if ((e = hipMalloc((void**)&scratch, fold_bytes + folds_bytes + packs_bytes)) != hipSuccess) return bail("hipMalloc jobs", e);
    float* fold = (float*)scratch;
    BNRef* folds_d = (BNRef*)(scratch + fold_bytes);
    Job* packs_d = (Job*)(scratch + fold_bytes + folds_bytes);
    if ((e = hipMemsetAsync(m, 0, I.total, st)) != hipSuccess) return bail("hipMemsetAsync", e);
    if ((e = hipMemcpyAsync(folds_d, J.folds.data(), J.folds.size() * sizeof(BNRef), hipMemcpyHostToDevice, st)) != hipSuccess ||
        (e = hipMemcpyAsync(packs_d, J.packs.data(), packs_bytes, hipMemcpyHostToDevice, st)) != hipSuccess)
        return bail("jobs", e);
    size_t most = 1;
    for (const Job& j : J.packs) most = std::max(most, j.count());
    hipLaunchKernelGGL(fold_kernel, dim3((unsigned)J.folds.size()), dim3(256), 0, st, folds_d, d_blob, fold);
    hipLaunchKernelGGL(pack_kernel, dim3((unsigned)std::min<size_t>((most + 255) / 256, 4096), (unsigned)J.packs.size()), dim3(256),
                       0, st, packs_d, d_blob, fold, m);
    if ((e = hipGetLastError()) != hipSuccess) return bail("pack kernels", e);
    if ((e = hipEventRecord(e1, st)) != hipSuccess || (e = hipStreamSynchronize(st)) != hipSuccess) return bail("roll sync", e);
    float ms = 0.f;
    (void)hipEventElapsedTime(&ms, e0, e1);
    net->last_roll_ms = ms;
    cleanup();
    *mp = m;
    *Ip = I;
    return 0;
}

extern "C" int gz_net_set_weights_device(gz_net* net, const float* d_blob, size_t count) {
    if (check_count(net, d_blob, count)) return -1;
    if (getenv("GZ_HOST_WEIGHT_ROLL")) {
        std::vector<float> h(count);
        HIPCHK(hipSetDevice(net->device));
        HIPCHK(hipMemcpy(h.data(), d_blob, count * 4, hipMemcpyDeviceToHost));
        return gz_net_set_weights(net, h.data(), count);
    }
    char *m = nullptr, *sm = nullptr;
    ImageLayout I, sI;
    if (build_image_device(net, d_blob, count, &m, &I)) return -1;
    if (gz_net* s = shadow_of(net)) {
        if (build_image_device(s, d_blob, count, &sm, &sI)) {
            (void)hipFree(m);
            return fail("shadow: " + g_err);
        }
    }
    return install_image(net, m, I, sm, &sI);
}


extern "C" double gz_net_last_roll_ms(const gz_net* net) { return net ? (double)net->last_roll_ms : -1.0; }

extern "C" size_t gz_net_copy_weight_image(gz_net* net, void* out, size_t cap) {
    if (!net || !net->dmem) return 0;
    std::lock_guard<std::mutex> wl(net->wmu);
    if (!out) return net->image_bytes;
    const size_t n = std::min(cap, net->image_bytes);
    if (hipSetDevice(net->device) != hipSuccess || hipDeviceSynchronize() != hipSuccess ||
        hipMemcpy(out, net->dmem, n, hipMemcpyDeviceToHost) != hipSuccess)
        return 0;
    return n;
}

static int launch_net(gz_net* net, hipStream_t stream, const gz_segment* segs, int nseg, hipEvent_t mid, int* rows) {
    *rows = 0;
    if (nseg < 1 || nseg > kMaxSegments) return fail("segment count out of range (1.." + std::to_string(kMaxSegments) + ")");
    if (!net->has_weights) return fail("weights not set");
    KParams kp = net->kp;
    int n = 0;
    for (int i = 0; i < nseg; ++i) {
        if (segs[i].rows < 0) return fail("negative segment rows");
        Segment& g = kp.seg[i];
        g.row0 = n;
        g.planes = segs[i].planes;
        for (int r = 0; r < kp.R; ++r) g.pol[r] = segs[i].policies[r];
        g.val = segs[i].values;
        n += segs[i].rows;
    }
    if (n <= 0) return 0;
    *rows = n;
    kp.n = n;
    kp.nseg = nseg;
    kp.stamps = net->stamps_on ? net->d_stamps : nullptr;
    {
        std::lock_guard<std::mutex> lk(net->feat_mu);
        auto& f = net->feat[stream];
        if (f.second < n) {
            if (f.first) {
                HIPCHK(hipDeviceSynchronize());
                HIPCHK(hipFree(f.first));
                f.first = nullptr;
            }
            const int cap = std::max(n, 8192);
            HIPCHK(hipMalloc((void**)&f.first, (size_t)cap * kp.FS * sizeof(float)));
            f.second = cap;
        }
        kp.feat = f.first;
        kp.glog = nullptr;
        if (net->gemm_heads) {
            auto& g = net->glog[stream];
            if (g.second < n) {
                if (g.first) {
                    HIPCHK(hipDeviceSynchronize());
                    HIPCHK(hipFree(g.first));
                    g.first = nullptr;
                }
                const int cap = std::max(n, 8192);
                HIPCHK(hipMalloc((void**)&g.first, (size_t)cap * kp.plog * sizeof(float)));
                g.second = cap;
            }
            kp.glog = g.first;
        }
    }
    if (net->fp32 || net->layered) {
        gzfp32::Forward f;
        f.parts = net->layered;
        if (net->fp32) {
            f.w0 = net->w0f;
            f.wres = net->wresf;
        }
        f.CP = net->in_width();
        f.FP = net->fpad;
        f.chunk_rows = net->chunk_rows;
        {
            std::lock_guard<std::mutex> lk(net->feat_mu);
            auto& s = net->fscr[stream];
            const int need = std::min(n, net->chunk_rows);
            if (s.second < need) {
                if (s.first) {
                    HIPCHK(hipDeviceSynchronize());
                    HIPCHK(hipFree(s.first));
                    s.first = nullptr;
                    s.second = 0;
                }
                const int cap = std::max(need, std::min(net->chunk_rows, 64));
                HIPCHK(hipMalloc((void**)&s.first, gzfp32::scratch_layout(cap, kp.npos, f.CP, f.FP).total));
                s.second = cap;
                if (net->f16) {
                    int*& be = net->bexp[stream];
                    if (be) HIPCHK(hipFree(be));
                    be = nullptr;
                    HIPCHK(hipMalloc((void**)&be, (size_t)cap * sizeof(int)));
                }
            }
            if (net->f16) f.bexp = net->bexp[stream];
            f.scratch = s.first;
            f.scratch_rows = s.second;
            f.scratch_bytes = gzfp32::scratch_layout(s.second, kp.npos, f.CP, f.FP).total;
        }
        if (f.scratch_bytes > gzfp32::kScratchMax) return fail("internal: fp32 scratch over its limit");
        if (const char* e = gzfp32::forward(kp, f, stream)) return fail(e);
        if (mid) HIPCHK(hipEventRecord(mid, stream));
        void* hargs[] = {&kp};
        if (net->gemm_heads) {
            int maxjt = 0;
            for (int r = 0; r < kp.R; ++r) maxjt = std::max(maxjt, (kp.P[r] + 15) / 16);
            HIPCHK(hipLaunchKernel((const void*)&policy_gemm_kernel, dim3((n + 63) / 64, (maxjt + 7) / 8, kp.R), dim3(256),
                                   hargs, 0, stream));
        }
        HIPCHK(hipLaunchKernel(net->fp32 || net->f16 ? (const void*)&heads_kernel_blocked : (const void*)&heads_kernel,
                               dim3((n + kHeadBoards - 1) / kHeadBoards), dim3(256), hargs, net->heads_smem, stream));
        return 0;
    }
    const gz_net::Trunk& t = n >= net->large_min_rows ? net->large : net->small;
    kp.resid = nullptr;
    if (t.resid_bytes) {
        std::lock_guard<std::mutex> lk(net->feat_mu);
        auto& f = net->resid[stream];
        const size_t need = (size_t)((n + t.nb - 1) / t.nb) * t.resid_bytes;
        if (f.second < need) {
            if (f.first) {
                HIPCHK(hipDeviceSynchronize());
                HIPCHK(hipFree(f.first));
                f.first = nullptr;
            }
            const size_t cap = std::max(need, (size_t)1024 * t.resid_bytes);
            HIPCHK(hipMalloc((void**)&f.first, cap));
            f.second = cap;
        }
        kp.resid = (f32x4*)f.first;
    }
    kp.btab_off = t.btab_off;
    kp.se_off = t.se_off;
    kp.cal_off = t.cal_off;
    void* args[] = {&kp};
    HIPCHK(hipLaunchKernel(t.fn, dim3((n + t.nb - 1) / t.nb), dim3(t.threads), args, t.smem, stream));
    if (mid) HIPCHK(hipEventRecord(mid, stream));
    if (net->gemm_heads) {
        int maxjt = 0;
        for (int r = 0; r < kp.R; ++r) maxjt = std::max(maxjt, (kp.P[r] + 15) / 16);
        HIPCHK(hipLaunchKernel((const void*)&policy_gemm_kernel, dim3((n + 63) / 64, (maxjt + 7) / 8, kp.R), dim3(256),
                               args, 0, stream));
    }
    if (!t.fused_heads)
        HIPCHK(hipLaunchKernel((const void*)&heads_kernel, dim3((n + kHeadBoards - 1) / kHeadBoards), dim3(256), args,
                               net->heads_smem, stream));
    return 0;
}

static int shadow_check(gz_net* net, hipStream_t stream, const gz_segment* segs, int nseg, int n) {
    std::lock_guard<std::mutex> sl(net->shadow_mu);
    gz_net::Shadow* sh = net->shadow;
    const long index = sh->forwards++;
    gz_net* s = sh->net;
    if (index % sh->every != 0 || !s->has_weights) return 0;
    const gz_net_desc& d = net->d;
    const int R = d.role_count, V = d.num_values, k = std::min(n, sh->max_rows);
    size_t out_f = V;
    for (int r = 0; r < R; ++r) out_f += d.policy_dist_count[r];
    gz_net::Shadow::Out& o = sh->out[stream];
    if (!o.out) {
        const size_t out_bytes = ((size_t)sh->max_rows * out_f * sizeof(float) + 15) & ~(size_t)15;
        HIPCHK(hipMalloc((void**)&o.out, out_bytes + (size_t)sh->max_rows * sizeof(gzshadow::RowRecord)));
        o.rec = (gzshadow::RowRecord*)((char*)o.out + out_bytes);
    }
    shadow_harvest(sh);
    gz_net::Shadow::Slot& slot = sh->slot[sh->next];
    if (slot.pending) shadow_harvest(sh, sh->next);
    if (sh->last_slot >= 0 && sh->last_stream != stream && sh->slot[sh->last_slot].pending)
        HIPCHK(hipStreamWaitEvent(stream, sh->slot[sh->last_slot].e1, 0));
    HIPCHK(hipEventRecord(slot.e0, stream));
    gz_segment ss[GZ_MAX_SEGMENTS];
    gzshadow::CompareArgs ca{};
    float* pol_b[GZ_MAX_ROLES];
    float* p = o.out;
    for (int r = 0; r < R; ++r) {
        pol_b[r] = p;
        p += (size_t)sh->max_rows * d.policy_dist_count[r];
        ca.pol_b[r] = pol_b[r];
        ca.P[r] = d.policy_dist_count[r];
    }
    ca.val_b = p;
    int m = 0, row0 = 0;
    for (int i = 0; i < nseg && row0 < k; ++i) {
        if (segs[i].rows <= 0) continue;
        gz_segment& g = ss[m];
        g = segs[i];
        g.rows = std::min(segs[i].rows, k - row0);
        ca.seg[m].row0 = row0;
        for (int r = 0; r < R; ++r) {
            ca.seg[m].pol[r] = segs[i].policies[r];
            g.policies[r] = pol_b[r] + (size_t)row0 * d.policy_dist_count[r];
        }
        ca.seg[m].val = segs[i].values;
        g.values = p + (size_t)row0 * V;
        row0 += g.rows;
        ++m;
    }
    int srows = 0;
    if (launch_net(s, stream, ss, m, nullptr, &srows)) return fail("shadow: " + g_err);
    ca.nseg = m;
    ca.n = k;
    ca.R = R;
    ca.V = V;
    ca.logits = net->kp.logits;
    ca.rec = o.rec;
    if (const char* e = gzshadow::launch_compare(ca, index, sh->fresh ? 1 : 0, sh->d_acc, stream)) return fail(std::string("shadow: ") + e);
    sh->fresh = false;
    HIPCHK(hipMemcpyAsync(slot.host, sh->d_acc, sizeof(gz_shadow_stats), hipMemcpyDeviceToHost, stream));
    HIPCHK(hipEventRecord(slot.e1, stream));
    slot.pending = true;
    slot.epoch = sh->epoch;
    sh->last_slot = sh->next;
    sh->last_stream = stream;
    sh->next = (sh->next + 1) % gz_net::Shadow::kSlots;
    return 0;
}

static int launch_segments(gz_net* net, hipStream_t stream, const gz_segment* segs, int nseg,
                           hipEvent_t mid = nullptr, hipEvent_t end = nullptr, unsigned long long* epoch = nullptr) {
    std::lock_guard<std::mutex> wl(net->wmu);
    if (epoch) *epoch = net->wepoch;
    int n = 0;
    if (launch_net(net, stream, segs, nseg, mid, &n)) return -1;
    if (end) HIPCHK(hipEventRecord(end, stream));
    if (n > 0 && net->shadow) return shadow_check(net, stream, segs, nseg, n);
    return 0;
}

static int launch(gz_net* net, hipStream_t stream, const float* d_planes, int n,
                  float* const* d_pol, float* d_val, hipEvent_t end = nullptr) {
    gz_segment sg{};
    sg.rows = n;
    sg.planes = d_planes;
    for (int r = 0; r < net->kp.R; ++r) sg.policies[r] = d_pol[r];
    sg.values = d_val;
    return launch_segments(net, stream, &sg, 1, nullptr, end);
}

extern "C" int gz_net_forward_device(gz_net* net, void* stream, const float* d_planes, int n,
                                     float* const* d_policies, float* d_values) {
    if (!net) return fail("null net");
    return launch(net, (hipStream_t)stream, d_planes, n, d_policies, d_values);
}

extern "C" int gz_net_forward_segments(gz_net* net, void* stream, const gz_segment* segs, int nseg) {
    if (!net || !segs) return fail("null argument");
    return launch_segments(net, (hipStream_t)stream, segs, nseg);
}

extern "C" int gz_net_forward_segments_ev(gz_net* net, void* stream, const gz_segment* segs, int nseg,
                                          void* trunk_done_event) {
    if (!net || !segs) return fail("null argument");
    return launch_segments(net, (hipStream_t)stream, segs, nseg, (hipEvent_t)trunk_done_event);
}

extern "C" int gz_net_forward(gz_net* net, const float* planes, int n, float* const* policies, float* values) {
    if (!net || !planes || !policies || !values) return fail("null argument");
    if (n <= 0) return 0;
    const gz_net_desc& d = net->d;
    const size_t in_f = (size_t)d.input_channels * d.input_columns * d.input_rows;
    size_t out_f = d.num_values;
    for (int r = 0; r < d.role_count; ++r) out_f += d.policy_dist_count[r];
    HIPCHK(hipSetDevice(net->device));
    if (n > net->io_cap) {
        if (net->d_io) HIPCHK(hipFree(net->d_io));
        net->d_io = nullptr;
        HIPCHK(hipMalloc((void**)&net->d_io, (size_t)n * (in_f + out_f) * 4 + 1024));
        net->io_cap = n;
    }
    float* d_in = net->d_io;
    float* d_pol[GZ_MAX_ROLES];
    float* p = d_in + (size_t)n * in_f;
    for (int r = 0; r < d.role_count; ++r) { d_pol[r] = p; p += (size_t)n * d.policy_dist_count[r]; }
    float* d_val = p;
    HIPCHK(hipMemcpyAsync(d_in, planes, (size_t)n * in_f * 4, hipMemcpyHostToDevice, net->stream));
    const bool stamps = getenv("GZ_KERNEL_STAMPS") != nullptr;
    const int grid = n;
    if (stamps && grid > net->stamp_cap) {
        if (net->d_stamps) HIPCHK(hipFree(net->d_stamps));
        HIPCHK(hipMalloc((void**)&net->d_stamps, (size_t)grid * 8 * sizeof(unsigned long long)));
        net->stamp_cap = grid;
    }
    if (stamps) HIPCHK(hipMemsetAsync(net->d_stamps, 0, (size_t)grid * 8 * sizeof(unsigned long long), net->stream));
    HIPCHK(hipEventRecord(net->ev0, net->stream));
    net->stamps_on = stamps;
    const int lrc = launch(net, net->stream, d_in, n, d_pol, d_val, net->ev1);
    net->stamps_on = false;
    if (lrc) return -1;
    for (int r = 0; r < d.role_count; ++r)
        HIPCHK(hipMemcpyAsync(policies[r], d_pol[r], (size_t)n * d.policy_dist_count[r] * 4, hipMemcpyDeviceToHost, net->stream));
    HIPCHK(hipMemcpyAsync(values, d_val, (size_t)n * d.num_values * 4, hipMemcpyDeviceToHost, net->stream));
    HIPCHK(hipStreamSynchronize(net->stream));
    HIPCHK(hipEventElapsedTime(&net->last_ms, net->ev0, net->ev1));
    if (stamps) {
        std::vector<unsigned long long> h((size_t)grid * 8);
        HIPCHK(hipMemcpy(h.data(), net->d_stamps, h.size() * sizeof(unsigned long long), hipMemcpyDeviceToHost));
        for (int i = 0; i < 8; ++i) net->stamp_avg[i] = 0;
        int wgs = 0;
        for (int b = 0; b < grid; ++b) {
            if (h[(size_t)b * 8] == 0 || h[(size_t)b * 8 + 4] == 0) continue;
            ++wgs;
            for (int i = 1; i < 5; ++i) net->stamp_avg[i] += (double)(h[(size_t)b * 8 + i] - h[(size_t)b * 8 + i - 1]);
        }
        for (int i = 1; i < 5; ++i) net->stamp_avg[i] = wgs ? net->stamp_avg[i] / wgs : 0.0;
        net->stamp_avg[0] = wgs;
    }
    return 0;
}

extern "C" int gz_net_stamp_avg(const gz_net* net, double* out8) {
    if (net && (net->fp32 || net->layered))
        return fail("no kernel stamps in the fp32-ieee and layered modes (the trunk is many launches)");
    for (int i = 0; i < 8; ++i) out8[i] = net->stamp_avg[i];
    return 0;
}

extern "C" float gz_net_last_kernel_ms(const gz_net* net) { return net ? net->last_ms : 0.f; }

extern "C" int gz_net_set_output_logits(gz_net* net, int on) {
    if (!net) return fail("null net");
    std::lock_guard<std::mutex> wl(net->wmu);
    if (net->kp.logits != (on ? 1 : 0)) ++net->wepoch;
    net->kp.logits = on ? 1 : 0;
    if (net->shadow) net->shadow->net->kp.logits = net->kp.logits;
    return 0;
}

void gzsym::net_view(gz_net* net, gzsym::NetView* out) {
    std::lock_guard<std::mutex> wl(net->wmu);
    const gz_net_desc& d = net->d;
    out->device = net->device;
    out->plane_elems = d.input_channels * d.input_columns * d.input_rows;
    out->roles = d.role_count;
    out->num_values = d.num_values;
    for (int r = 0; r < GZ_MAX_ROLES; ++r) out->policy[r] = r < d.role_count ? d.policy_dist_count[r] : 0;
    out->logits = net->kp.logits;
    out->host_stream = net->stream;
}

int gzsym::set_error(const std::string& msg) { return fail(msg); }

unsigned long long gzcache::net_epoch(gz_net* net) {
    std::lock_guard<std::mutex> wl(net->wmu);
    return net->wepoch;
}

int gzcache::forward_segments_epoch(gz_net* net, void* stream, const gz_segment* segs, int nseg, unsigned long long* epoch) {
    return launch_segments(net, (hipStream_t)stream, segs, nseg, nullptr, nullptr, epoch);
}

extern "C" int gz_nn_compare_outputs(int device, int n, int roles, const int* policy_sizes, int num_values,
                                     const float* const* pol_a, const float* val_a, const float* const* pol_b,
                                     const float* val_b, gz_shadow_stats* out) {
    if (!policy_sizes || !pol_a || !val_a || !pol_b || !val_b || !out) return fail("null argument");
    if (n < 1 || roles < 1 || roles > GZ_MAX_ROLES || num_values < 1 || num_values > 4) return fail("compare: sizes out of range");
    size_t row_f = num_values;
    for (int r = 0; r < roles; ++r) {
        if (policy_sizes[r] < 1 || !pol_a[r] || !pol_b[r]) return fail("compare: bad policy array");
        row_f += policy_sizes[r];
    }
    HIPCHK(hipSetDevice(device));
    const size_t side = ((size_t)n * row_f * sizeof(float) + 15) & ~(size_t)15;
    const size_t recs = (size_t)n * sizeof(gzshadow::RowRecord);
    char* mem = nullptr;
    hipStream_t st = nullptr;
    hipEvent_t e0 = nullptr, e1 = nullptr;
    hipError_t e = hipMalloc((void**)&mem, 2 * side + recs + sizeof(gz_shadow_stats));
    if (e == hipSuccess) e = hipStreamCreateWithFlags(&st, hipStreamNonBlocking);
    if (e == hipSuccess) e = hipEventCreate(&e0);
    if (e == hipSuccess) e = hipEventCreate(&e1);
    gzshadow::CompareArgs ca{};
    ca.nseg = 1;
    ca.n = n;
    ca.R = roles;
    ca.V = num_values;
    ca.rec = (gzshadow::RowRecord*)(mem + 2 * side);
    gz_shadow_stats* d_acc = (gz_shadow_stats*)(mem + 2 * side + recs);
    const char* cmp_err = nullptr;
    if (e == hipSuccess) {
        for (int sd = 0; sd < 2 && e == hipSuccess; ++sd) {
            float* p = (float*)(mem + sd * side);
            for (int r = 0; r < roles && e == hipSuccess; ++r) {
                const size_t cnt = (size_t)n * policy_sizes[r];
                e = hipMemcpyAsync(p, (sd ? pol_b : pol_a)[r], cnt * sizeof(float), hipMemcpyHostToDevice, st);
                if (sd) ca.pol_b[r] = p; else ca.seg[0].pol[r] = p;
                ca.P[r] = policy_sizes[r];
                p += cnt;
            }
            if (e == hipSuccess) e = hipMemcpyAsync(p, sd ? val_b : val_a, (size_t)n * num_values * sizeof(float), hipMemcpyHostToDevice, st);
            if (sd) ca.val_b = p; else ca.seg[0].val = p;
        }
        if (e == hipSuccess) e = hipEventRecord(e0, st);
        if (e == hipSuccess) cmp_err = gzshadow::launch_compare(ca, 0, 1, d_acc, st);
        if (e == hipSuccess && !cmp_err) e = hipEventRecord(e1, st);
        if (e == hipSuccess && !cmp_err) e = hipMemcpyAsync(out, d_acc, sizeof(gz_shadow_stats), hipMemcpyDeviceToHost, st);
        const hipError_t es = hipStreamSynchronize(st);
        if (e == hipSuccess) e = es;
        float ms = 0.f;
        if (e == hipSuccess && !cmp_err) e = hipEventElapsedTime(&ms, e0, e1);
        if (e == hipSuccess && !cmp_err) out->device_ms = ms;
    }
    if (e0) (void)hipEventDestroy(e0);
    if (e1) (void)hipEventDestroy(e1);
    if (st) (void)hipStreamDestroy(st);
    if (mem) (void)hipFree(mem);
    if (cmp_err) return fail(cmp_err);
    if (e != hipSuccess) return fail(std::string("gz_nn_compare_outputs: ") + hipGetErrorString(e));
    return 0;
}

extern "C" int gz_net_large_min_rows(const gz_net* net) { return net ? net->large_min_rows : 0; }

extern "C" const char* gz_net_kernel_name(const gz_net* net, int large) {
    if (!net) return "";
    return (large ? net->large : net->small).name.c_str();
}

extern "C" int gz_net_wave_rows(const gz_net* net) {
    if (!net) return 0;
    if (net->fp32 || net->layered) {
        const int gy = net->fpad / (32 * gzfp32::wave_co_tiles(net->fpad));
        return std::max(1, (kCUs / gy) * gzfp32::kTileCols / net->kp.npos);
    }
    const gz_net::Trunk& t = net->large_min_rows < (1 << 30) ? net->large : net->small;
    return t.nb * t.wgs_per_cu * kCUs;
}

extern "C" int gz_net_workgroups_per_cu(const gz_net* net) {
    if (!net || net->fp32 || net->layered) return 1;
    return (net->large_min_rows < (1 << 30) ? net->large : net->small).wgs_per_cu;
}
```

### galvanise_zero_amd/csrc/nn/trunk_variants.h

```cpp
#pragma once

#include "forward_kernel.h"

#include <cstdio>

namespace gznn {

struct KernelChoice {
    const void* fn = nullptr;
    int act_bytes = 0;
    int nb = 1;
    bool single_image = false;
    int resid_bytes = 0;
    int threads = 256;
    int groups = 1;
    bool in_place = false;
    int wgs_per_cu = 1;
    char name[64] = {0};
};

template <int F, int PTN, int NB, int WPE, int P = 1, bool V2 = false>
KernelChoice kernel_for() {
    KernelChoice k;
    if constexpr (V2) k.fn = (const void*)&trunk_kernel_v2<F, PTN, NB, WPE, P>;
    else k.fn = (const void*)&trunk_kernel<F, PTN, NB, WPE, P>;
    k.act_bytes = Geo<F, PTN, NB, P>::ACT_BYTES;
    k.nb = NB;
    k.single_image = Geo<F, PTN, NB, P>::SI;
    k.resid_bytes = Geo<F, PTN, NB, P>::RESID_BYTES + Geo<F, PTN, NB, P>::LO_BYTES;
    std::snprintf(k.name, sizeof(k.name), "gznn::trunk_kernel%s<%d, %d, %d, %d, %d>", V2 ? "_v2" : "", F, PTN, NB, WPE, P);
    return k;
}

template <int F, int PTN, int P>
KernelChoice kernel8_for() {
    KernelChoice k;
    k.fn = (const void*)&trunk_kernel8<F, PTN, P>;
    k.act_bytes = Geo<F, PTN, 1, P, 2>::ACT_BYTES;
    k.nb = 2;
    k.threads = 512;
    k.groups = 2;
    std::snprintf(k.name, sizeof(k.name), "gznn::trunk_kernel8<%d, %d, %d>", F, PTN, P);
    return k;
}

template <int F, int PTN, int P>
KernelChoice kernelw8_for() {
    KernelChoice k;
    k.fn = (const void*)&trunk_kernel_w8<F, PTN, P>;
    k.act_bytes = Geo<F, PTN, 2, P, 3>::ACT_BYTES;
    k.nb = 2;
    k.threads = 512;
    std::snprintf(k.name, sizeof(k.name), "gznn::trunk_kernel_w8<%d, %d, %d>", F, PTN, P);
    return k;
}

template <int F, int PTN, int P>
KernelChoice kernelh2_for() {
    KernelChoice k;
    k.fn = (const void*)&trunk_kernel_h2<F, PTN, P>;
    k.act_bytes = Geo<F, PTN, 1, P, 4>::ACT_BYTES;
    k.nb = 2;
    k.groups = 2;
    std::snprintf(k.name, sizeof(k.name), "gznn::trunk_kernel_h2<%d, %d, %d>", F, PTN, P);
    return k;
}

template <int F, int PTN, int P>
KernelChoice kernelh2i_for() {
    KernelChoice k;
    k.fn = (const void*)&trunk_kernel_h2i<F, PTN, P>;
    k.act_bytes = Geo<F, PTN, 1, P, 5>::ACT_BYTES;
    k.nb = 2;
    k.groups = 2;
    k.in_place = true;
    k.wgs_per_cu = 2;
    std::snprintf(k.name, sizeof(k.name), "gznn::trunk_kernel_h2i<%d, %d, %d>", F, PTN, P);
    return k;
}

template <int F, int PTN, bool V2 = false>
KernelChoice variants(int v, int precision) {
    if (precision == 3) {
        if constexpr (F == 256) {
            if constexpr (Geo<F, PTN, 1, 3>::SI && Geo<F, PTN, 1, 3>::ACT_BYTES + 40 * 1024 <= 160 * 1024 &&
                          !Geo<F, PTN, 1, 3>::RG) {
                if (v == 11) return kernel_for<F, PTN, 1, 1, 3, V2>();
            } else if constexpr (Geo<F, PTN, 1, 2>::SI && Geo<F, PTN, 1, 2>::ACT_BYTES + 16 * 1024 <= 160 * 1024) {
                if (v == 11) return kernel_for<F, PTN, 1, 1, 2, V2>();
            }
            return KernelChoice{};
        }
        if constexpr (F <= 128 && PTN > 4) {
            if (v == 11) return kernel_for<F, PTN, 1, 1, 2, V2>();
            return KernelChoice{};
        }
        if constexpr (F <= 128 && PTN <= 4) {
            if constexpr (2 * Geo<F, PTN, 1, 3>::ACT_BYTES + 16 * 1024 <= 160 * 1024) {
                if (v == 11) return kernel_for<F, PTN, 1, 1, 3, V2>();
                if constexpr (Geo<F, PTN, 1, 3>::WRAP && 4 * Geo<F, PTN, 1, 3>::ACT_BYTES + 16 * 1024 <= 160 * 1024) {
                    if (v == 21) return kernel_for<F, PTN, 2, 1, 3, V2>();
                    if constexpr (!V2) {
                        if (v == 22) return kernel8_for<F, PTN, 3>();
                        if constexpr (F == 128) {
                            if (v == 24) return kernelw8_for<F, PTN, 3>();
                            if (v == 23) return kernelh2_for<F, PTN, 3>();
                            if (v == 25) return kernelh2i_for<F, PTN, 3>();
                        }
                    }
                }
            }
        }
        return KernelChoice{};
    }
    if constexpr (4 * Geo<F, PTN, 1>::ACT_BYTES + 16 * 1024 > 160 * 1024) {
        return v == 11 ? kernel_for<F, PTN, 1, 1, 1, V2>() : KernelChoice{};
    } else {
        switch (v) {
            case 11: return kernel_for<F, PTN, 1, 1, 1, V2>();
            case 12: if constexpr (PTN == 4) return kernel_for<F, PTN, 1, 2, 1, V2>(); else return KernelChoice{};
            case 21:
                if constexpr (Geo<F, PTN, 2>::LIVE_VGPRS <= 300) return kernel_for<F, PTN, 2, 1, 1, V2>();
                else return KernelChoice{};
            default: return KernelChoice{};
        }
    }
}

KernelChoice trunk_variant_f64(int pt, int v, int precision);
KernelChoice trunk_variant_f128(int pt, int v, int precision);
KernelChoice trunk_variant_f256(int pt, int v, int precision);
KernelChoice trunk_variant_f64_v2(int pt, int v, int precision);
KernelChoice trunk_variant_f128_v2(int pt, int v, int precision);
KernelChoice trunk_variant_f256_v2(int pt, int v, int precision);

inline int padded_filters(int F) { return F <= 64 ? 64 : F <= 128 ? 128 : F <= 256 ? 256 : 0; }
constexpr int kMaxPT = 23;
constexpr int kLargePT = 23;
inline int kernel_tiles(int pt) { return pt > 11 && pt <= kLargePT ? kLargePT : pt; }
inline int kernel_filters(int F, int pt) {
    const int f = padded_filters(F);
    return pt > 11 && f == 64 ? 128 : f;
}

inline KernelChoice trunk_variant(int fpad, int pt, int v, int precision, bool v2 = false) {
    if (v2) {
        if (fpad == 64) return trunk_variant_f64_v2(pt, v, precision);
        if (fpad == 128) return trunk_variant_f128_v2(pt, v, precision);
        if (fpad == 256) return trunk_variant_f256_v2(pt, v, precision);
        return KernelChoice{};
    }
    if (fpad == 64) return trunk_variant_f64(pt, v, precision);
    if (fpad == 128) return trunk_variant_f128(pt, v, precision);
    if (fpad == 256) return trunk_variant_f256(pt, v, precision);
    return KernelChoice{};
}

}
```

Measured before the change: 2.426 million.

## Pair board rows across two images in the in-place split kernel to skip edge taps

```diff
diff --git a/galvanise_zero_amd/csrc/nn/forward_kernel.h b/galvanise_zero_amd/csrc/nn/forward_kernel.h
--- a/galvanise_zero_amd/csrc/nn/forward_kernel.h
+++ b/galvanise_zero_amd/csrc/nn/forward_kernel.h
@@ -4,6 +4,8 @@
 #include <stdint.h>
 
 #include <utility>
+
+#include "rowpair.h"
 
 namespace gznn {
 
@@ -108,6 +110,7 @@
 __host__ __device__ constexpr int gcd_c(int a, int b) { return b == 0 ? a : gcd_c(b, a % b); }
 __host__ __device__ constexpr int lcm_c(int a, int b) { return a / gcd_c(a, b) * b; }
 
+__host__ __device__ constexpr bool wg_in_place(int wg) { return wg == 5 || wg == 6; }
 template <int F, int PTN, int NB = 1, int P = 1, int WG = 1>
 struct Geo {
     static constexpr int P2 = P == 3 ? 2 : 1;
@@ -115,8 +118,8 @@
     static constexpr int NPOS = 16 * PTN;
     static constexpr int PT = PTN;
     static constexpr int TT = NB * PT;
-    static constexpr int NWV = WG == 3 ? 8 : (WG == 4 || WG == 5) ? 2 : 4;
-    static constexpr int NGR = WG == 2 || WG == 4 || WG == 5 ? 2 : 1;
+    static constexpr int NWV = WG == 3 ? 8 : (WG == 4 || wg_in_place(WG)) ? 2 : 4;
+    static constexpr int NGR = WG == 2 || WG == 4 || wg_in_place(WG) ? 2 : 1;
     static constexpr int CT = F / (16 * NWV);
     static constexpr int KC = F / 32;
     static constexpr int CPR = F / 8;
@@ -129,8 +132,8 @@
     static constexpr int NFR = CT * WP;
     static constexpr int ROWB = 64 * WP;
     static constexpr int NST = 9 * KC / KS;
-    static constexpr int R0 = (P2 == 2 && (NB == 2 || WG == 2 || WG == 4 || WG == 5) && (KC / KS) >= 3 && NST % (KC / KS) == 0 &&
-                               (KC / KS) * KS * NFR * 4 <= (WG == 4 ? GZ_H2_RING_VGPRS : WG == 5 ? 64 : 96))
+    static constexpr int R0 = (P2 == 2 && (NB == 2 || WG == 2 || WG == 4 || wg_in_place(WG)) && (KC / KS) >= 3 && NST % (KC / KS) == 0 &&
+                               (KC / KS) * KS * NFR * 4 <= (WG == 4 ? GZ_H2_RING_VGPRS : wg_in_place(WG) ? 64 : 96))
                                   ? KC / KS
                                   : ring_depth(NST, KS, NFR, CT >= 4 ? 64 : 96);
     static constexpr int LIVE_VGPRS = R0 * KS * NFR * 4 + 2 * TT * P2 * 4 + 2 * CT * TT * 4;
@@ -140,12 +143,17 @@
     static constexpr bool LOOPSI = (kLoopSI || PTN > 11) && SI && NST % US == 0 && NST / US >= 2;
     static constexpr int R = LOOPSI ? RS : R0;
     static constexpr int LPS = KS * NFR;
-    static constexpr bool INPL = WG == 5;
+    static constexpr bool INPL = wg_in_place(WG);
+    static constexpr bool RP = WG == 5 && PTN == kRowPairTiles;
+    static constexpr int IMG_STRIDE = ACT_BYTES + (RP ? kRowPairPad : 0);
+    static_assert(!RP || (ROWS == kRowPairRowBytes && HALF == kRowPairHalf && ACT_BYTES == kRowPairImage && ZROWS == 2 &&
+                          IMG_STRIDE == kRowPairStride && NPOS == kRowPairSide * kRowPairSide),
+                  "row pairs: rowpair.h's image");
     static constexpr bool RG = CT * TT * 4 * 2 > 256;
-    static constexpr bool TRACKED = SI || LIVE_VGPRS > 300 || (P2 == 2 && (NB == 2 || WG == 2 || WG == 4 || WG == 5));
+    static constexpr bool TRACKED = SI || LIVE_VGPRS > 300 || (P2 == 2 && (NB == 2 || WG == 2 || WG == 4 || wg_in_place(WG)));
     static_assert(F % 64 == 0, "filters must be a multiple of 64");
     static_assert(!SI || NB == 1, "single-image mode takes one board per workgroup");
-    static_assert(WG == 1 || ((WG == 2 || WG == 4 || WG == 5) && NB == 1 && !SI) || (WG == 3 && !SI && CT >= 1),
+    static_assert(WG == 1 || ((WG == 2 || WG == 4 || wg_in_place(WG)) && NB == 1 && !SI) || (WG == 3 && !SI && CT >= 1),
                   "wave groups: two images, or one in place (INPL), never the single-image conv and heads");
     static_assert(!INPL || (P == 3 && WRAP), "in place: the split F = 128 kernels");
     static_assert(!RG || SI, "the global residual is implemented for single-image kernels");
@@ -304,9 +312,14 @@
 struct TapAddr {
     int row, rot;
 };
-template <int F, int PTN, int P = 1>
-__device__ __forceinline__ TapAddr tap_base(int tap, int pt, int lane, const Board& bd) {
+template <int F, int PTN, int P = 1, bool RP = false>
+__device__ __forceinline__ TapAddr tap_base(int tap, int pt, int lane, const Board& bd, int rset = 0) {
     using G = Geo<F, PTN, 1, P>;
+    if constexpr (RP) {
+        using GR = Geo<F, PTN, 1, P, 5>;
+        static_assert(GR::RP && G::WRAP, "row pairs: the in-place split kernel at four tiles");
+        return TapAddr{rowpair_tap_offset<G::ROWS, GR::IMG_STRIDE>(rset, pt, lane, tap), 0};
+    }
     const int li = lane & 15, g = lane >> 4;
     const int dy = tap / 3 - 1, dx = tap % 3 - 1;
     const int p = 16 * pt + li;
@@ -473,10 +486,12 @@
                                              f32x4 (&acc)[Geo<F, PTN, NB, P, WG>::CT][Geo<F, PTN, NB, P, WG>::TT],
                                              bf16x8 (&b)[Geo<F, PTN, NB, P, WG>::TT][Geo<F, PTN, NB, P, WG>::P2],
                                              const __bf16* wres, uint32_t woff, int gs_it, int gmax, int& lane,
-                                             const Board& bd, int tap0, bool last_it, const Epi& epi = Epi{}) {
+                                             const Board& bd, int tap0, bool last_it, const Epi& epi, int rset, bool skip0,
+                                             bool rd0, int (&tb)[Geo<F, PTN, NB, P, WG>::PT]) {
     using G = Geo<F, PTN, NB, P, WG>;
     constexpr int R = G::R, KS = G::KS, CT = G::CT, PT = G::PT, KC = G::KC, P2 = G::P2, WP = G::WP;
     static_assert(P != 2 || G::TRACKED, "two-pass split: compiler-tracked weight loads");
+    static_assert(!G::RP || (G::TPI == 1 && !EPI && NB == 1), "row pairs: one tap per iteration");
     static_assert(G::U % R == 0, "ring slots must be static within an iteration");
     if constexpr (P == 2) {
         constexpr int SLOT = (ST + R - 1) % R;
@@ -503,13 +518,27 @@
         const int tap = tap0 + jn / KC, kc = jn % KC;
         if (kc == 0) launder(lane);
         int nb_off[PT];
-#pragma unroll
-        for (int pt = 0; pt < PT; ++pt) nb_off[pt] = tap_offset<F, PTN, P>(tap_base<F, PTN, P>(tap, pt, lane, bd), kc);
+        if constexpr (G::RP) {
+            if (kc == 0) {
+#pragma unroll
+                for (int pt = 0; pt < PT; ++pt) {
+                    if (pt == 0 && !rd0) continue;
+                    tb[pt] = tap_base<F, PTN, P, true>(tap, pt, lane, bd, rset).row;
+                    launder(tb[pt]);
+                }
+            }
+#pragma unroll
+            for (int pt = 0; pt < PT; ++pt) nb_off[pt] = tb[pt] + 64 * kc;
+        } else {
+#pragma unroll
+            for (int pt = 0; pt < PT; ++pt) nb_off[pt] = tap_offset<F, PTN, P>(tap_base<F, PTN, P>(tap, pt, lane, bd), kc);
+        }
 #pragma unroll
         for (int bb = 0; bb < NB; ++bb)
 #pragma unroll
             for (int pt = 0; pt < PT; ++pt) {
                 const int t = bb * PT + pt;
+                if (!(G::RP && t == 0) || !skip0)
 #pragma unroll
                 for (int ct = 0; ct < CT; ++ct) {
                     const bf16x8 w_hi = ring.r[ST % R][k][ct * WP];
@@ -525,8 +554,10 @@
                 }
                 {
                     const char* a = X + nb_off[pt] + bb * G::ACT_BYTES;
-#pragma unroll
-                    for (int h = 0; h < P2; ++h) b[t][h] = *(const bf16x8*)(a + h * G::HALF);
+                    if (!(G::RP && t == 0) || (kc != 0 ? !skip0 : rd0)) {
+#pragma unroll
+                        for (int h = 0; h < P2; ++h) b[t][h] = *(const bf16x8*)(a + h * G::HALF);
+                    }
                 }
                 if constexpr (P2 == 1) {
                     __builtin_amdgcn_sched_group_barrier(0x008, CT * (P == 2 && PASS == 0 ? 2 : 1), 0);
@@ -554,17 +585,17 @@
                                           f32x4 (&acc)[Geo<F, PTN, NB, P, WG>::CT][Geo<F, PTN, NB, P, WG>::TT],
                                           bf16x8 (&b)[Geo<F, PTN, NB, P, WG>::TT][Geo<F, PTN, NB, P, WG>::P2],
                                           const __bf16* wres, uint32_t woff, int gs_it, int gmax, int& lane,
-                                          const Board& bd, int tap0, bool last_it, const Epi& epi,
-                                          std::integer_sequence<int, ST...>) {
+                                          const Board& bd, int tap0, bool last_it, const Epi& epi, int rset, bool skip0,
+                                          bool rd0, int (&tb)[Geo<F, PTN, NB, P, WG>::PT], std::integer_sequence<int, ST...>) {
     (conv_stage_l<F, PTN, NB, P, WG, PASS, ST, EPI, Epi>(X, ring, acc, b, wres, woff, gs_it, gmax, lane, bd, tap0, last_it,
-                                                         epi), ...);
+                                                         epi, rset, skip0, rd0, tb), ...);
 }
 
 template <int F, int PTN, int NB, int P, int WG = 1, int PASS = 0, bool EPI = false, class Epi = NoEpi>
 __device__ __forceinline__ void conv3x3_looped(const char* __restrict__ X, Ring<F, PTN, NB, P, WG>& ring,
                                                f32x4 (&acc)[Geo<F, PTN, NB, P, WG>::CT][Geo<F, PTN, NB, P, WG>::TT],
                                                const __bf16* wres, uint32_t woff, int gs0, int gmax, int lane,
-                                               const Board& bd, const Epi& epi = Epi{}) {
+                                               const Board& bd, const Epi& epi = Epi{}, int rset = 0) {
     using G = Geo<F, PTN, NB, P, WG>;
     constexpr int PT = G::PT, TT = G::TT;
     if constexpr (PASS == 0) {
@@ -574,26 +605,54 @@
             for (int t = 0; t < TT; ++t) acc[ct][t] = f32x4{0.f, 0.f, 0.f, 0.f};
     }
     bf16x8 b[TT][G::P2];
+    int tb[PT];
     launder(lane);
-#pragma unroll
-    for (int pt = 0; pt < PT; ++pt) {
-        const char* a = X + tap_offset<F, PTN, P>(tap_base<F, PTN, P>(0, pt, lane, bd), 0);
-#pragma unroll
-        for (int bb = 0; bb < NB; ++bb)
-#pragma unroll
-            for (int h = 0; h < G::P2; ++h) b[bb * PT + pt][h] = *(const bf16x8*)(a + bb * G::ACT_BYTES + h * G::HALF);
-    }
-    if constexpr (G::P2 == 2) split_chain_enter(acc);
-    constexpr int NLOOP = EPI ? G::NIT - 1 : G::NIT;
+    if constexpr (G::RP) {
+        static_assert(G::TPI == 1 && G::NIT == 9 && !EPI && NB == 1, "row pairs: one tap per iteration");
+#pragma unroll
+        for (int pt = 0; pt < PT; ++pt) {
+            tb[pt] = tap_base<F, PTN, P, true>(0, pt, lane, bd, rset).row;
+            launder(tb[pt]);
+            const char* a = X + tb[pt];
+            if (pt != 0 || !rowpair_skip(rset, 0, 0)) {
+#pragma unroll
+                for (int h = 0; h < G::P2; ++h) b[pt][h] = *(const bf16x8*)(a + h * G::HALF);
+            }
+        }
+        split_chain_enter(acc);
+        static_assert(rowpair_skip(0, 0, 0) && rowpair_skip(0, 0, 2) && !rowpair_skip(0, 0, 3) && !rowpair_skip(1, 0, 5) &&
+                      rowpair_skip(1, 0, 6) && rowpair_skip(1, 0, 8) && !rowpair_skip(1, 0, 9), "the short taps");
+        const int first_short = rset == 0 ? 0 : 6;
 #pragma clang loop unroll(disable)
-    for (int it = 0; it < NLOOP; ++it)
-        conv_iter<F, PTN, NB, P, WG, PASS, false, NoEpi>(X, ring, acc, b, wres, woff, gs0 + it * G::U, gmax, lane, bd,
-                                                       it * G::TPI, it == G::NIT - 1, NoEpi{},
-                                                       std::make_integer_sequence<int, G::U>{});
-    if constexpr (EPI)
-        conv_iter<F, PTN, NB, P, WG, PASS, true, Epi>(X, ring, acc, b, wres, woff, gs0 + NLOOP * G::U, gmax, lane, bd,
-                                                   NLOOP * G::TPI, true, epi, std::make_integer_sequence<int, G::U>{});
-    if constexpr (G::P2 == 2) split_chain_leave(acc);
+        for (int it = 0; it < G::NIT; ++it)
+            conv_iter<F, PTN, NB, P, WG, PASS, false, NoEpi>(X, ring, acc, b, wres, woff, gs0 + it * G::U, gmax, lane, bd, it,
+                                                             it == G::NIT - 1, NoEpi{}, rset,
+                                                             (unsigned)(it - first_short) < 3u,
+                                                             !((unsigned)(it + 1 - first_short) < 3u), tb,
+                                                             std::make_integer_sequence<int, G::U>{});
+        split_chain_leave(acc);
+    } else {
+#pragma unroll
+        for (int pt = 0; pt < PT; ++pt) {
+            const char* a = X + tap_offset<F, PTN, P>(tap_base<F, PTN, P>(0, pt, lane, bd), 0);
+#pragma unroll
+            for (int bb = 0; bb < NB; ++bb)
+#pragma unroll
+                for (int h = 0; h < G::P2; ++h) b[bb * PT + pt][h] = *(const bf16x8*)(a + bb * G::ACT_BYTES + h * G::HALF);
+        }
+        if constexpr (G::P2 == 2) split_chain_enter(acc);
+        constexpr int NLOOP = EPI ? G::NIT - 1 : G::NIT;
+#pragma clang loop unroll(disable)
+        for (int it = 0; it < NLOOP; ++it)
+            conv_iter<F, PTN, NB, P, WG, PASS, false, NoEpi>(X, ring, acc, b, wres, woff, gs0 + it * G::U, gmax, lane, bd,
+                                                             it * G::TPI, it == G::NIT - 1, NoEpi{}, 0, false, true, tb,
+                                                             std::make_integer_sequence<int, G::U>{});
+        if constexpr (EPI)
+            conv_iter<F, PTN, NB, P, WG, PASS, true, Epi>(X, ring, acc, b, wres, woff, gs0 + NLOOP * G::U, gmax, lane, bd,
+                                                          NLOOP * G::TPI, true, epi, 0, false, true, tb,
+                                                          std::make_integer_sequence<int, G::U>{});
+        if constexpr (G::P2 == 2) split_chain_leave(acc);
+    }
 }
 
 template <int F, int PTN, int NB, int P, int WG = 1>
@@ -759,11 +818,13 @@
     constexpr int IP2 = G::WP;
     constexpr int PT = G::PT, TT = G::TT, CT = G::CT, R = G::R, NWV = G::NWV, NGR = G::NGR, kThreads = 64 * NWV;
     const int NPOS = kp.npos, H = kp.H, W = kp.W;
+    const int grp = NGR == 1 ? 0 : __builtin_amdgcn_readfirstlane((int)(threadIdx.x / kThreads));
     Board bd{H, W, NPOS, kp.wmagic, {}};
     {
         const int li = threadIdx.x & 15;
 #pragma unroll
         for (int pt = 0; pt < PT; ++pt) {
+            if constexpr (G::RP) continue;
             const int p = 16 * pt + li;
             const int r = bd.row(p), x = p - r * W;
             int m = 0;
@@ -779,8 +840,7 @@
 
     constexpr bool SI = G::SI, RG = G::RG;
     extern __shared__ __attribute__((aligned(16))) char smem[];
-    const int grp = NGR == 1 ? 0 : __builtin_amdgcn_readfirstlane((int)(threadIdx.x / kThreads));
-    char* X0 = smem + grp * NB * ACT;
+    char* X0 = smem + grp * NB * G::IMG_STRIDE;
     constexpr bool INPL = G::INPL;
     char* X1 = SI ? smem : INPL ? X0 : smem + NGR * NB * ACT + grp * NB * ACT;
     char* SCR = X1;
@@ -796,6 +856,19 @@
     const int wave = __builtin_amdgcn_readfirstlane(tid >> 6);
     const int g = lane >> 4, li = lane & 15;
     const int co_base = wave * (F / NWV);
+    auto tile_img = [&](char* Xg, int t, int li_) -> char* {
+        if constexpr (G::RP) return smem + (li_ >> 3) * G::IMG_STRIDE;
+        else return Xg + (t / PT) * ACT;
+    };
+    auto tile_pos = [&](int t, int li_) -> int {
+        if constexpr (G::RP) return rowpair_map(grp, t, li_).pos;
+        else return 16 * (t % PT) + li_;
+    };
+    auto li_now = [&]() -> int {
+        int v = li;
+        if constexpr (G::RP) launder(v);
+        return v;
+    };
     const int C = kp.C, K0 = kp.K0;
 
     constexpr int kPF = 4;
@@ -933,9 +1006,9 @@
             if (s + 1 < nk0) load_w0(s + 1, an, alon);
 #pragma unroll
             for (int pt = 0; pt < PT; ++pt) {
-                const int p = 16 * pt + li;
+                const int p = tile_pos(pt, li);
                 const int q = p < NPOS ? p : NPOS;
-                const int o = q * imrow + ((((s * 4 + g)) ^ (q & imswz)) << 4);
+                const int o = q * imrow + ((((s * 4 + g)) ^ (q & imswz)) << 4) + (G::RP ? ((li >> 3) - grp) * G::IMG_STRIDE : 0);
                 const bf16x8 bq = *(const bf16x8*)(IM + o);
 #pragma unroll
                 for (int ct = 0; ct < CT; ++ct) {
@@ -993,7 +1066,8 @@
                     }
                 }
             }
-        } else
+        } else {
+        const int lie = li_now();
 #pragma unroll
         for (int ct = 0; ct < CT; ++ct) {
             const int co = co_base + 16 * ct + 4 * g;
@@ -1021,9 +1095,11 @@
                     store_act<F, PTN, 1, false>(X0 + bb * ACT, 16 * pt + li, co, sv, NPOS);
                     store_lo_scratch<F, PTN>(xlo, 16 * pt + li, co, sv, NPOS);
                 } else {
-                    store_act<F, PTN, P, !G::SI>(X0 + bb * ACT, 16 * pt + li, co, preact ? pre_act(v, psc, psh, kp.leaky) : v, NPOS);
-                }
-            }
+                    store_act<F, PTN, P, !G::SI>(tile_img(X0, bb * PT + pt, lie), tile_pos(pt, lie), co,
+                                                 preact ? pre_act(v, psc, psh, kp.leaky) : v, NPOS);
+                }
+            }
+        }
         }
         if constexpr (V2)
             if (kp.cal) cal_partial(0, bb, li, g);
@@ -1155,6 +1231,7 @@
         const float* b_b = b_a + F;
 
         static_assert(!(INPL && kEpiInConv), "an epilogue inside the conv writes the other image");
+        static_assert(!(G::RP && (V2 || !G::LOOP)), "row pairs: the v1 looped conv");
         if constexpr (!V2 && G::LOOP && kEpiInConv) {
             float4 bia[CT];
 #pragma unroll
@@ -1193,9 +1270,10 @@
             __syncthreads();
             continue;
         }
-        if constexpr (G::LOOP) conv3x3_looped<F, PTN, NB, P, WG>(X0, ring, acc, kp.wres, woff, (2 * blk) * G::NST, gmax, lane, bd);
+        if constexpr (G::LOOP) conv3x3_looped<F, PTN, NB, P, WG>(G::RP ? smem : X0, ring, acc, kp.wres, woff, (2 * blk) * G::NST, gmax, lane, bd, NoEpi{}, grp);
         else conv3x3<F, PTN, NB, P, WG>(X0, ring, acc, kp.wres, woff, (2 * blk) * G::NST, gmax, lane, bd);
         if constexpr (INPL) __syncthreads();
+        const int lia = li_now();
 #pragma unroll
         for (int ct = 0; ct < CT; ++ct) {
             const int co = co_base + 16 * ct + 4 * g;
@@ -1207,12 +1285,12 @@
                 v[1] = act_mx(v[1] + bias.y, alpha);
                 v[2] = act_mx(v[2] + bias.z, alpha);
                 v[3] = act_mx(v[3] + bias.w, alpha);
-                store_act<F, PTN, P, !G::SI>(X1 + (t / PT) * ACT, 16 * (t % PT) + li, co, v, NPOS);
+                store_act<F, PTN, P, !G::SI>(tile_img(X1, t, lia), tile_pos(t, lia), co, v, NPOS);
             }
         }
         __syncthreads();
 
-        if constexpr (G::LOOP) conv3x3_looped<F, PTN, NB, P, WG>(X1, ring, acc, kp.wres, woff, (2 * blk + 1) * G::NST, gmax, lane, bd);
+        if constexpr (G::LOOP) conv3x3_looped<F, PTN, NB, P, WG>(G::RP ? smem : X1, ring, acc, kp.wres, woff, (2 * blk + 1) * G::NST, gmax, lane, bd, NoEpi{}, grp);
         else conv3x3<F, PTN, NB, P, WG>(X1, ring, acc, kp.wres, woff, (2 * blk + 1) * G::NST, gmax, lane, bd);
         if constexpr (INPL) __syncthreads();
         if constexpr (V2) {
@@ -1251,6 +1329,7 @@
             if (kp.cal) cal_reduce(blk + 1);
             continue;
         }
+        const int lib = li_now();
 #pragma unroll
         for (int ct = 0; ct < CT; ++ct) {
             const int co = co_base + 16 * ct + 4 * g;
@@ -1265,7 +1344,7 @@
                 v[3] = act_mx(v[3] + bias.w + r[3], alpha);
                 resid[ct][t] = v;
                 acc[ct][t] = v;
-                store_act<F, PTN, P, !G::SI>(X0 + (t / PT) * ACT, 16 * (t % PT) + li, co, v, NPOS);
+                store_act<F, PTN, P, !G::SI>(tile_img(X0, t, lib), tile_pos(t, lib), co, v, NPOS);
             }
         }
         __syncthreads();
@@ -1291,7 +1370,7 @@
 
     GZ_STAMP(2);
     int lih = li, gh = g;
-    if constexpr (V2 && SI) {
+    if constexpr ((V2 && SI) || G::RP) {
         launder(lih);
         launder(gh);
     }
@@ -1322,7 +1401,7 @@
 #pragma unroll
     for (int bb = 0; bb < NB; ++bb) {
         const int board = board0 + bb;
-        if (kp.gapF && board < kp.n) {
+        if (!G::RP && kp.gapF && board < kp.n) {
             const float inv = 1.f / (float)NPOS;
 #pragma unroll
             for (int ct = 0; ct < CT; ++ct) {
@@ -1335,9 +1414,11 @@
             }
         }
         auto head_conv = [&](int h, const float4 (&wv)[CT]) {
+            float* hp = hpart;
+            if constexpr (G::RP) hp = (float*)tile_img(SCR, 0, lih);
 #pragma unroll
             for (int pt = 0; pt < PT; ++pt) {
-                const int p = 16 * pt + lih;
+                const int p = tile_pos(pt, lih);
 #pragma unroll
                 for (int ct = 0; ct < CT; ++ct) {
                     const f32x4 a = acc[ct][bb * PT + pt];
@@ -1347,7 +1428,7 @@
                     s += a[3] * wv[ct].w;
                     s += __shfl_xor(s, 16, 64);
                     s += __shfl_xor(s, 32, 64);
-                    if (gh == 0 && p < NPOS) hpart[((bb * NT16 + co_base / 16 + ct) * HC + h) * NPOS + p] = s;
+                    if (gh == 0 && p < NPOS) hp[((bb * NT16 + co_base / 16 + ct) * HC + h) * NPOS + p] = s;
                 }
             }
         };
@@ -1423,6 +1504,11 @@
 __global__ void __launch_bounds__(256) __attribute__((amdgpu_waves_per_eu(2)))
 trunk_kernel_h2i(const KParams kp) {
     trunk_body<F, PTN, 1, 2, P, false, 5>(kp);
+}
+template <int F, int PTN, int P>
+__global__ void __launch_bounds__(256) __attribute__((amdgpu_waves_per_eu(2)))
+trunk_kernel_h2ig(const KParams kp) {
+    trunk_body<F, PTN, 1, 2, P, false, 6>(kp);
 }
 
 template <int F, int PTN, int NB, int WPE, int P>
diff --git a/galvanise_zero_amd/csrc/nn/gz_nn.hip b/galvanise_zero_amd/csrc/nn/gz_nn.hip
--- a/galvanise_zero_amd/csrc/nn/gz_nn.hip
+++ b/galvanise_zero_amd/csrc/nn/gz_nn.hip
@@ -119,11 +119,15 @@
 
 constexpr int kSmallVariant = 11, kLargeVariant = 23, kLargeFallback = 21, kLargeMinRows = 257;
 constexpr int kLargeInPlace = 25;
+constexpr int kInPlaceGeneric = 26;
 constexpr int kCUs = 256;
 
-static KernelChoice select_kernel(int fpad, int pt, int v, int precision, bool v2) {
+static KernelChoice select_kernel(const gz_net_desc& d, int fpad, int pt, int v, int precision, bool v2) {
     if (pt < 1 || pt > kMaxPT) return KernelChoice{};
-    return trunk_variant(fpad, pt, v, precision, v2);
+    KernelChoice k = trunk_variant(fpad, pt, v, precision, v2);
+    if (k.fn && k.square8 && (d.input_columns != 8 || d.input_rows != 8 || gap_features(d)))
+        k = trunk_variant(fpad, pt, kInPlaceGeneric, precision, v2);
+    return k;
 }
 
 static gz_net* create_host(const gz_net_desc& d, int device, gz_net::Trunk* in_place) {
@@ -165,9 +169,9 @@
         }
         min_large = 1 << 30;
     }
-    KernelChoice kc = layerwise ? KernelChoice{} : select_kernel(fpad, pt, vs, precision, v2);
-    KernelChoice kl = layerwise ? KernelChoice{} : select_kernel(fpad, pt, vl, precision, v2);
-    if (!kl.fn && vl == kLargeVariant) kl = select_kernel(fpad, pt, kLargeFallback, precision, v2);
+    KernelChoice kc = layerwise ? KernelChoice{} : select_kernel(d, fpad, pt, vs, precision, v2);
+    KernelChoice kl = layerwise ? KernelChoice{} : select_kernel(d, fpad, pt, vl, precision, v2);
+    if (!kl.fn && vl == kLargeVariant) kl = select_kernel(d, fpad, pt, kLargeFallback, precision, v2);
     auto wg_fits = [&](const KernelChoice& c) {
         if (c.groups == 1) return true;
         const int np = d.input_columns * d.input_rows;
@@ -179,12 +183,12 @@
                                  gap_features(d), c.nb, 1, fpad) <= c.act_bytes;
     };
     if (kl.fn && !wg_fits(kl)) {
-        kl = vl == kLargeVariant ? select_kernel(fpad, pt, kLargeFallback, precision, v2) : KernelChoice{};
+        kl = vl == kLargeVariant ? select_kernel(d, fpad, pt, kLargeFallback, precision, v2) : KernelChoice{};
         if (kl.fn && !wg_fits(kl)) kl = KernelChoice{};
     }
     if (kc.fn && !wg_fits(kc)) kc = KernelChoice{};
     KernelChoice ki = !layerwise && getenv("GZ_KERNEL_VARIANT") == nullptr && kl.fn
-                          ? select_kernel(fpad, pt, kLargeInPlace, precision, v2) : KernelChoice{};
+                          ? select_kernel(d, fpad, pt, kLargeInPlace, precision, v2) : KernelChoice{};
     if (ki.fn && !wg_fits(ki)) ki = KernelChoice{};
     if (kc.fn && !kl.fn && vl != vs) {
         kl = kc;
@@ -228,7 +232,7 @@
                                                                            c.groups == 2 ? 1 : c.nb, fpad))
                                       : scr_in;
         t.btab_off = c.single_image ? align16(std::max(c.act_bytes, scr))
-                     : c.in_place   ? c.nb * c.act_bytes
+                     : c.in_place   ? c.nb * c.act_bytes + c.img_pad
                                     : c.nb * c.act_bytes + std::max(c.nb * c.act_bytes, scr);
         t.resid_bytes = c.resid_bytes;
         t.smem = t.btab_off + bias_table_bytes(fpad, d.residual_layers);
diff --git a/galvanise_zero_amd/csrc/nn/rowpair.h b/galvanise_zero_amd/csrc/nn/rowpair.h
--- /dev/null
+++ b/galvanise_zero_amd/csrc/nn/rowpair.h
@@ -0,0 +1,44 @@
+#pragma once
+
+#if defined(__HIPCC__) || defined(__CUDACC__)
+#define GZ_RP_HD __host__ __device__
+#else
+#define GZ_RP_HD
+#endif
+
+namespace gznn {
+
+constexpr int kRowPairSide = 8;
+constexpr int kRowPairTiles = 4;
+constexpr int kRowPairPad = 160;
+constexpr int kRowPairRowBytes = 544, kRowPairHalf = 256, kRowPairImage = 67 * kRowPairRowBytes;
+constexpr int kRowPairStride = kRowPairImage + kRowPairPad;
+
+struct RowPairPos {
+    int board, pos;
+};
+
+GZ_RP_HD constexpr int rowpair_row(int set, int t) { return set == 0 ? t : kRowPairSide - 1 - t; }
+
+GZ_RP_HD constexpr RowPairPos rowpair_map(int set, int t, int li) {
+    return RowPairPos{li >> 3, kRowPairSide * rowpair_row(set, t) + (li & 7)};
+}
+
+GZ_RP_HD constexpr bool rowpair_skip(int set, int t, int tap) {
+    return t == 0 && (set == 0 ? tap < 3 : (tap >= 6 && tap < 9));
+}
+
+template <int ROWS, int STRIDE>
+GZ_RP_HD inline int rowpair_tap_offset(int set, int t, int lane, int tap) {
+    static_assert(STRIDE % 256 == 0, "the two boards' lanes of a tile would share LDS slots");
+    const int x = lane & 7, board = (lane >> 3) & 1, g = lane >> 4;
+    const int tp = tap > 8 ? 4 : tap;
+    const int xx = x + tp % 3 - 1;
+    const int y = rowpair_row(set, t) + tp / 3 - 1;
+    const bool ok = (unsigned)xx < (unsigned)kRowPairSide && (unsigned)y < (unsigned)kRowPairSide;
+    const int a_in = (kRowPairSide * y + xx) * ROWS + (g << 4);
+    const int a_zero = kRowPairSide * kRowPairSide * ROWS + (((g + 2 * xx) & 15) << 4);
+    return board * STRIDE + (ok ? a_in : a_zero);
+}
+
+}
diff --git a/galvanise_zero_amd/csrc/nn/trunk_variants.h b/galvanise_zero_amd/csrc/nn/trunk_variants.h
--- a/galvanise_zero_amd/csrc/nn/trunk_variants.h
+++ b/galvanise_zero_amd/csrc/nn/trunk_variants.h
@@ -16,6 +16,8 @@
     int groups = 1;
     bool in_place = false;
     int wgs_per_cu = 1;
+    int img_pad = 0;
+    bool square8 = false;
     char name[64] = {0};
 };
 
@@ -75,7 +77,22 @@
     k.groups = 2;
     k.in_place = true;
     k.wgs_per_cu = 2;
+    k.img_pad = Geo<F, PTN, 1, P, 5>::IMG_STRIDE - Geo<F, PTN, 1, P, 5>::ACT_BYTES;
+    k.square8 = Geo<F, PTN, 1, P, 5>::RP;
     std::snprintf(k.name, sizeof(k.name), "gznn::trunk_kernel_h2i<%d, %d, %d>", F, PTN, P);
+    return k;
+}
+
+template <int F, int PTN, int P>
+KernelChoice kernelh2ig_for() {
+    KernelChoice k;
+    k.fn = (const void*)&trunk_kernel_h2ig<F, PTN, P>;
+    k.act_bytes = Geo<F, PTN, 1, P, 6>::ACT_BYTES;
+    k.nb = 2;
+    k.groups = 2;
+    k.in_place = true;
+    k.wgs_per_cu = 2;
+    std::snprintf(k.name, sizeof(k.name), "gznn::trunk_kernel_h2ig<%d, %d, %d>", F, PTN, P);
     return k;
 }
 
@@ -106,6 +123,9 @@
                             if (v == 24) return kernelw8_for<F, PTN, 3>();
                             if (v == 23) return kernelh2_for<F, PTN, 3>();
                             if (v == 25) return kernelh2i_for<F, PTN, 3>();
+                            if constexpr (Geo<F, PTN, 1, 3, 5>::RP) {
+                                if (v == 26) return kernelh2ig_for<F, PTN, 3>();
+                            }
                         }
                     }
                 }
```

Result: faster. 2.452 million (median of 6 runs) (+1.0%).
